# maybeLx/MVSFormerPlusPlus

Hardware: NVIDIA H100
Metric: depth-maps/sec (hot path: FMT + 4-stage cascade) (higher is better)
Workload: dtype f32

## Files before the change

include/mvsf_b200.h:

```cpp
#ifndef MVSF_B200_H
#define MVSF_B200_H

#include <stddef.h>
#include <stdint.h>

#ifdef __cplusplus
extern "C" {
#endif

typedef void* mvsf_stream_t;

enum mvsf_status {
  MVSF_OK = 0,
  MVSF_ERR_INVALID = -1,
  MVSF_ERR_CUDA = -2,
  MVSF_ERR_WORKSPACE = -3
};

const char* mvsf_last_error(void);
int mvsf_abi_version(void);
long long mvsf_launch_count(int reset);
int mvsf_ktimer_enable(int on);
int mvsf_ktimer_read(const char* name, double* ms, long long* launches);

int mvsf_nchw_to_nhwc(const float* src, float* dst, int N, int C, int HW, mvsf_stream_t stream);
int mvsf_nhwc_to_nchw(const float* src, float* dst, int N, int C, int HW, mvsf_stream_t stream);

int mvsf_compose_geometry(const float* proj, int V, float* homs, float* kinv_ref, mvsf_stream_t stream);

int mvsf_homography_from_proj(const float* src_proj, const float* ref_proj, int B, float* homs, mvsf_stream_t stream);

int mvsf_init_inverse_range(const float* depth_values, int Dn, float* out, int D, int H, int W, mvsf_stream_t stream);
int mvsf_schedule_inverse_range(const float* prev_depth, const float* prev_hypo, int Dp, float split_itv, float* out,
                                int D, int H, int W, mvsf_stream_t stream);
int mvsf_position3d(const float* kinv_ref, const float* depth, const float* depth_values, int Dn, float* stats,
                    int compute_minmax, float* pos, int D, int H, int W, mvsf_stream_t stream);

int mvsf_homo_warp(const float* src_nhwc, const float* hom, const float* depth, float* warped, uint8_t* mask, int C,
                   int D, int H, int W, mvsf_stream_t stream);

int mvsf_warp_corr_set_tile_path(int mode);
int mvsf_warp_corr_last_selection(int* used_pipeline, int* miss_permille);

int mvsf_warp_corr_plan(int C, int G, int D, int H, int W, int V, size_t spill_budget_bytes);

int mvsf_warp_corr_entropy(const float* feat, const float* homs, const float* depth, float* entropy, int V, int C,
                           int G, int D, int H, int W, mvsf_stream_t stream);
int mvsf_vis_cnn(const float* entropy, const float* wts, float* vis, int N, int H, int W, mvsf_stream_t stream);
int mvsf_warp_corr_aggregate(const float* feat, const float* homs, const float* depth, const float* vis,
                             float* volume, int V, int C, int G, int D, int H, int W, mvsf_stream_t stream);
int mvsf_warp_corr_entropy_store(const float* feat, const float* homs, const float* depth, float* entropy, float* corr,
                                 int V, int C, int G, int D, int H, int W, mvsf_stream_t stream);
int mvsf_corr_aggregate(const float* corr, const float* vis, float* volume, int V, int G, int D, int H, int W,
                        mvsf_stream_t stream);

int mvsf_costreg_unet_workspace_bytes(int kind, int C, int D, int H, int W, size_t* bytes);
int mvsf_costreg_unet_tc_bytes(size_t* bytes);
int mvsf_costreg_unet_pack_tc(int kind, const float* conv, void* wts_tc, size_t wts_tc_bytes, mvsf_stream_t stream);
int mvsf_costreg_unet_forward(int kind, const float* volume, const float* wts, const void* wts_tc, float* logits,
                              void* workspace, size_t workspace_bytes, int C, int D, int H, int W, mvsf_stream_t stream);
int mvsf_conv3d_tc_layer(int mode, int sd, const float* in, const float* w32, const float* skip, float* out,
                         void* workspace, size_t workspace_bytes, int cin, int cout, int ID, int IH, int IW,
                         mvsf_stream_t stream);

int mvsf_costreg_tr_workspace_bytes(int C, int D, int H, int W, size_t* bytes);
int mvsf_costreg_tr_forward(float* volume, const float* pos, const float* wts, const void* wts16, size_t n_wts,
                            float* logits, void* workspace, size_t workspace_bytes, int C, int D, int H, int W,
                            int layers, float softmax_scale, mvsf_stream_t stream);
int mvsf_split_weights_f16(const float* wts, void* out16, size_t n, mvsf_stream_t stream);

int mvsf_attention_forward(const float* qkv, float* out, void* workspace, size_t workspace_bytes, int N,
                           float softmax_scale, mvsf_stream_t stream);

int mvsf_attention_split_plan(int N, int num_sms, int* split_items, int* parts);

int mvsf_linear_tc_epilogue(int epi, const float* A, int lda, const float* W, const float* bias, const float* res,
                            int ldres, const float* gamma, const float* ln_w, const float* ln_b, float ln_eps,
                            int elu_cols, float* C, int ldc, float* Cpre, int ldcpre, void* C2, int ldc2,
                            void* workspace, size_t workspace_bytes, int M, int N, int K, mvsf_stream_t stream);
int mvsf_token_mlp_forward(int form, const float* A, const float* res, const float* proj_w, const float* proj_b,
                           const float* gamma1, const float* mid_w, const float* mid_b, float mid_eps, const float* f1_w,
                           const float* f1_b, const float* f2_w, const float* f2_b, const float* gamma2,
                           const float* out_w, const float* out_b, float out_eps, float* C, void* C2, void* workspace,
                           size_t workspace_bytes, int M, mvsf_stream_t stream);
int mvsf_linear_tc_streamed_epilogue(int epi, const float* A, int lda, const float* W, const float* bias,
                                     const float* res, int ldres, const float* gamma, int elu_cols, float* C, int ldc,
                                     void* C2, int ldc2, void* workspace, size_t workspace_bytes, int M, int N, int K,
                                     mvsf_stream_t stream);

int mvsf_softargmax(const float* logits, const float* depth_hypo, float tmp, float* prob, float* depth, float* conf,
                    int D, int H, int W, mvsf_stream_t stream);
int mvsf_conf_accumulate(const float* conf, int h, int w, float* acc, int H, int W, float scale, int init,
                         mvsf_stream_t stream);

int mvsf_fmt_workspace_bytes(int V, int H1, int W1, size_t* bytes);
int mvsf_fmt_forward(const float* f1, const float* f2, const float* f3, const float* f4, const float* pe,
                     const float* wts, const void* wts16, size_t n_wts, float* o1, float* o2, float* o3, float* o4,
                     void* workspace, size_t workspace_bytes, int V, int H1, int W1, mvsf_stream_t stream);

int mvsf_fpn_encoder_workspace_bytes(int N, int H, int W, size_t* bytes);
int mvsf_fpn_encoder_forward(const float* x, const float* wts, const void* wts_tc, float* c01, float* c11, float* c21,
                             float* c31, void* workspace, size_t workspace_bytes, int N, int H, int W, mvsf_stream_t stream);
int mvsf_fpn_encoder_vit_forward(const float* x, const float* vit_feat, int V, const float* wts, const void* wts_tc,
                                 float* c01, float* c11, float* c21, float* c31, void* workspace, size_t workspace_bytes,
                                 int N, int H, int W, mvsf_stream_t stream);
int mvsf_fpn_decoder_workspace_bytes(int N, int H, int W, size_t* bytes);
int mvsf_fpn_decoder_forward(const float* c01, const float* c11, const float* c21, const float* c31, const float* wts,
                             const void* wts_tc, float* o0, float* o1, float* o2, float* o3, void* workspace,
                             size_t workspace_bytes, int N, int H, int W, mvsf_stream_t stream);
int mvsf_fpn_tc_bytes(int part, size_t* bytes);
int mvsf_fpn_pack_tc(int part, const float* conv, void* wts_tc, size_t wts_tc_bytes, mvsf_stream_t stream);

int mvsf_vit_decoder_workspace_bytes(int B, int V, int h, int w, size_t* bytes);
int mvsf_vit_decoder_forward(const float* x0, const float* x1, const float* x2, const float* wts, const void* wts_tc,
                             float* out, void* workspace, size_t workspace_bytes, int B, int V, int h, int w,
                             mvsf_stream_t stream);

int mvsf_vit_workspace_bytes(int n, int gh, int gw, size_t* bytes);
int mvsf_vit_forward(const float* img, const float* pos, const float* wts, const void* wts_tc, float* out0, float* out1,
                     float* out2, void* workspace, size_t workspace_bytes, int n, int gh, int gw, mvsf_stream_t stream);
int mvsf_vit_forward_image(const float* img, int H, int W, const float* pos, const float* wts, const void* wts_tc,
                           float* out0, float* out1, float* out2, void* workspace, size_t workspace_bytes, int n, int gh,
                           int gw, mvsf_stream_t stream);
int mvsf_vit_attention_forward(const float* qkv, int ldq, float* out, int ldo, void* workspace, size_t workspace_bytes,
                               int n, int N, mvsf_stream_t stream);

int mvsf_fusion_workspace_bytes(int H, int W, size_t* bytes);
int mvsf_fusion_prepare_cameras(const float* cams, int N, float* cams_inv, mvsf_stream_t stream);
int mvsf_fusion_filter(int method, const float* depths, const float* confs, const float* cams, const float* cams_inv, int N,
                       int ref, const int* src, int V, int H, int W, float conf, float thres_view, float thres_disp,
                       float dist_base, float rel_diff_base, unsigned char* mask, float* depth_avg, void* workspace,
                       size_t workspace_bytes, mvsf_stream_t stream);
int mvsf_fusion_extract(const unsigned char* mask, const float* depth_avg, const void* workspace, size_t workspace_bytes,
                        const float* cam_inv, const float* image, float* xyz, unsigned char* rgb, long long capacity, int H,
                        int W, mvsf_stream_t stream);

#ifdef __cplusplus
}
#endif
#endif
```

mvsformerplusplus_b200/csrc/conv3d_tc.cu:

```cuda
#include "conv3d_tc.cuh"

#include <type_traits>

#include "linear_tc.cuh"
#include "wgmma.cuh"

namespace mvsf {

using namespace gmma;

namespace c3 {
constexpr int THREADS = 384, MAX_STAGES = 8;
template <int MODE, int NT>
struct Geo {
  static constexpr int TW = 8 * NT, TH = 16;
  static constexpr int PR = MODE == CONV_S1 ? TH + 2 : TH + 1;
  static constexpr int PC = MODE == CONV_S1 ? TW + 2 : TW + 1;
  static constexpr int NSUB = MODE == CONV_S2 ? 4 : 1;
  static constexpr uint32_t SUB_BYTES = PR * PC * 16;
  static constexpr uint32_t PAIR = (2 * SUB_BYTES + 127) / 128 * 128;
  static constexpr uint32_t OCT_BYTES = NSUB * PAIR;
  static constexpr uint32_t PITCH = PC * 16;
};
__host__ __device__ inline int npad(int cout) { return cout < 16 ? 16 : cout; }
__host__ __device__ inline uint32_t slab_bytes(int mode, int cout) { return (uint32_t)npad(cout) * (mode == DECONV_S2 ? 1024u : 576u); }

struct alignas(64) Maps { CUtensorMap m[4]; };
}

struct DepthTaps { int n, kd[3], id[3]; };
template <int MODE>
__device__ __forceinline__ DepthTaps depth_taps(int od, int SD, int ID) {
  DepthTaps t;
  t.n = 0;
#pragma unroll
  for (int kd = 0; kd < 3; ++kd) {
    int id;
    bool ok = true;
    if (MODE == CONV_S1) id = od + kd - 1;
    else if (MODE == CONV_S2) id = od * SD + kd - 1;
    else {
      const int num = od + 1 - kd;
      if (SD == 1) id = num;
      else { ok = (num & 1) == 0; id = num >> 1; }
    }
    if (ok && id >= 0 && id < ID) { t.kd[t.n] = kd; t.id[t.n] = id; ++t.n; }
  }
  return t;
}

template <int OUT, int NPAD>
__device__ __forceinline__ float conv_epilogue_frag(const ConvTcArgs& a, const float* acc, int h, int q, bool valid, size_t vox) {
  const int COUT = a.COUT;
  float prob = 0.f;
#pragma unroll
  for (int b = 0; b < NPAD / 8; ++b) {
    const int c = 8 * b + 2 * q;
    if (8 * b >= COUT) continue;
    const float2 b2 = *reinterpret_cast<const float2*>(a.bias + c);
    float x0 = fmaxf(acc[4 * b + 2 * h] + b2.x, 0.f), x1 = fmaxf(acc[4 * b + 2 * h + 1] + b2.y, 0.f);
    if (!valid) continue;
    if (OUT == OUT_SPLIT) {
      if (a.skip_hi) {
        const float2 fh = __half22float2(*reinterpret_cast<const __half2*>(a.skip_hi + vox * COUT + c));
        const float2 fl = __half22float2(*reinterpret_cast<const __half2*>(a.skip_lo + vox * COUT + c));
        x0 += fh.x + fl.x;
        x1 += fh.y + fl.y;
      }
      split_store2(a.out_hi + vox * COUT + c, a.out_lo + vox * COUT + c, x0, x1);
    } else {
      const float2 s2 = *reinterpret_cast<const float2*>(a.skip32 + vox * COUT + c);
      x0 += s2.x; x1 += s2.y;
      if (OUT == OUT_F32) *reinterpret_cast<float2*>(a.out32 + vox * COUT + c) = make_float2(x0, x1);
      else prob = fmaf(x1, __ldg(a.probw + c + 1), x0 * __ldg(a.probw + c));
    }
  }
  return prob;
}

template <int NREG>
__device__ __forceinline__ void fence_acc(float (&acc)[NREG]) { fence_regs<NREG>(acc); }

template <int MODE, int NT, int OUT, int NPAD>
__global__ void __launch_bounds__(c3::THREADS, 1)
conv3d_tc_kernel(const __grid_constant__ c3::Maps maps, ConvTcArgs a, int NS, int OD, int OH, int OW, int tiles_w,
                 int tiles_h, int ntiles) {
  using G = c3::Geo<MODE, NT>;
  constexpr int PC = G::PC, NSUB = G::NSUB;
  constexpr int NCLS = MODE == DECONV_S2 ? 4 : 1;
  constexpr int ACC = NCLS * NPAD / 2;
  extern __shared__ __align__(1024) unsigned char smem[];
  const int tid = threadIdx.x, warp = tid >> 5, lane = tid & 31;
  const int CIN = a.CIN, SD = a.SD, ID = a.ID, IH = a.IH, IW = a.IW;
  const int KG = a.KG;
  const uint32_t b_bytes = c3::slab_bytes(MODE, NPAD);
  const uint32_t a_bytes = (uint32_t)KG * G::OCT_BYTES;
  const uint32_t stage_bytes = (a_bytes + b_bytes + 127u) / 128u * 128u;
  const uint32_t sbase = smem_u32(smem);
  const uint32_t bars = sbase + NS * stage_bytes;
  const uint32_t bar_full = bars, bar_empty = bars + 64;
  const int ngroups = (CIN >> 3) / KG;

  if (tid == 0) {
    for (int i = 0; i < c3::MAX_STAGES; ++i) { mbar_init(bar_full + 8 * i, 1); mbar_init(bar_empty + 8 * i, 2); }
    fence_barrier_init();
  }
  __syncthreads();

  if (warp < 4) {
    asm volatile("setmaxnreg.dec.sync.aligned.u32 40;");
    if (tid == 0) {
      uint32_t g = 0;
      for (int tile = blockIdx.x; tile < ntiles; tile += gridDim.x) {
        const int tw = tile % tiles_w, th = (tile / tiles_w) % tiles_h, od = tile / (tiles_w * tiles_h);
        const int c0h = th * 16, c0w = tw * G::TW;
        const DepthTaps dt = depth_taps<MODE>(od, SD, ID);
        for (int ds = 0; ds < dt.n; ++ds) {
          for (int grp = 0; grp < ngroups; ++grp, ++g) {
            const int s = g % NS;
            mbar_wait(bar_empty + 8 * s, (uint32_t)(((g / NS) & 1) ^ 1));
            const uint32_t st = sbase + s * stage_bytes, full = bar_full + 8 * s;
            expect_tx(full, (uint32_t)(KG * NSUB) * 2u * G::SUB_BYTES + b_bytes);
            for (int og = 0; og < KG; ++og) {
              const int c = (grp * KG + og) * 8;
#pragma unroll
              for (int sub = 0; sub < NSUB; ++sub) {
                int w0, h0;
                if (MODE == CONV_S1) { w0 = c0w - 1; h0 = c0h - 1; }
                else if (MODE == CONV_S2) { w0 = c0w - (sub & 1); h0 = c0h - (sub >> 1); }
                else { w0 = c0w; h0 = c0h; }
                tma_load_5d(st + (uint32_t)(og * NSUB + sub) * G::PAIR, &maps.m[sub], c, w0, h0, dt.id[ds], 0, full);
              }
            }
            bulk_load(st + a_bytes, a.wtc + (size_t)(dt.kd[ds] * ngroups + grp) * (b_bytes / 2), b_bytes, full);
          }
        }
      }
    }
    return;
  }
  asm volatile("setmaxnreg.inc.sync.aligned.u32 232;");
  const int half = (warp >> 2) - 1, wq = warp & 3, q = lane & 3, t128 = tid & 127;
  const uint32_t blk = (uint32_t)NPAD * 32u;
  float acc[NT][ACC];
  auto release = [&](uint32_t gb) { if (t128 == 0) mbar_arrive(bar_empty + 8 * (gb % NS)); };
  uint32_t g = 0;
  for (int tile = blockIdx.x; tile < ntiles; tile += gridDim.x) {
    const int tw = tile % tiles_w, th = (tile / tiles_w) % tiles_h, od = tile / (tiles_w * tiles_h);
    const DepthTaps dt = depth_taps<MODE>(od, SD, ID);
    const int U = dt.n * ngroups;
    int pend = -1;
    for (int u = 0; u < U; ++u, ++g) {
      const int s = g % NS;
      mbar_wait(bar_full + 8 * s, (uint32_t)((g / NS) & 1));
      const uint32_t sA = sbase + s * stage_bytes + (uint32_t)half * 8u * G::PITCH, sB = sbase + s * stage_bytes + a_bytes;
      auto issue = [&](uint32_t aoff, int bstart, bool overwrite) {
        constexpr uint32_t n = (uint32_t)(NCLS * NPAD);
        const uint32_t t0 = sB + (uint32_t)bstart * 2u * blk, t1 = t0 + (uint32_t)NCLS * blk;
        const uint64_t b0 = make_desc(t0, n * 16u, 128), b1 = make_desc(t1, n * 16u, 128);
        if (KG == 1) {
#pragma unroll
          for (int t = 0; t < NT; ++t)
            mma_ss<n>(acc[t], make_desc(sA + aoff + t * 128, G::SUB_BYTES, G::PITCH), b0, overwrite ? 0u : 1u);
#pragma unroll
          for (int t = 0; t < NT; ++t)
            mma_ss<n>(acc[t], make_desc(sA + aoff + t * 128, G::SUB_BYTES, G::PITCH), b1, 1u);
        } else {
#pragma unroll
          for (int t = 0; t < NT; ++t)
            mma_ss<n>(acc[t], make_desc(sA + G::SUB_BYTES + aoff + t * 128, G::OCT_BYTES, G::PITCH), b0, overwrite ? 0u : 1u);
#pragma unroll
          for (int t = 0; t < NT; ++t)
            mma_ss<n>(acc[t], make_desc(sA + aoff + t * 128, G::OCT_BYTES, G::PITCH), b1, 1u);
#pragma unroll
          for (int t = 0; t < NT; ++t)
            mma_ss<n>(acc[t], make_desc(sA + aoff + t * 128, G::OCT_BYTES, G::PITCH), b0, 1u);
        }
      };
      wg_fence();
      if constexpr (MODE == DECONV_S2) {
        issue(0u, 0, u == 0);
        issue(16u, 4, false);
        issue((uint32_t)PC * 16u, 8, false);
        issue((uint32_t)(PC + 1) * 16u, 12, false);
      } else {
#pragma unroll
        for (int kh = 0; kh < 3; ++kh) {
#pragma unroll
          for (int kw = 0; kw < 3; ++kw) {
            int sub = 0, rs = kh, cs = kw;
            if (MODE == CONV_S2) {
              sub = (kh == 1 ? 0 : 2) + (kw == 1 ? 0 : 1);
              rs = kh == 2 ? 1 : 0; cs = kw == 2 ? 1 : 0;
            }
            issue((uint32_t)sub * G::PAIR + (uint32_t)(rs * PC + cs) * 16u, kh * 3 + kw, u == 0 && kh == 0 && kw == 0);
          }
        }
      }
      wg_commit();
      if (pend >= 0) {
        wg_wait<1>();
        release((uint32_t)pend);
      }
      pend = (int)g;
    }
    wg_wait<0>();
#pragma unroll
    for (int t = 0; t < NT; ++t) fence_acc(acc[t]);
    release((uint32_t)pend);
#pragma unroll
    for (int t = 0; t < NT; ++t)
#pragma unroll
      for (int cls = 0; cls < NCLS; ++cls)
#pragma unroll
        for (int h = 0; h < 2; ++h) {
          const int ch = th * 16 + 8 * half + 2 * wq + h;
          const int cw = tw * G::TW + t * 8 + (lane >> 2);
          int oh, ow;
          bool valid;
          if (MODE == DECONV_S2) { oh = 2 * ch + (cls >> 1); ow = 2 * cw + (cls & 1); valid = ch < IH && cw < IW; }
          else { oh = ch; ow = cw; valid = ch < OH && cw < OW; }
          const size_t vox = valid ? ((size_t)od * OH + oh) * OW + ow : 0;
          float prob = conv_epilogue_frag<OUT, NPAD>(a, acc[t] + (cls ^ (cls >> 1)) * (NPAD / 2), h, q, valid, vox);
          if (OUT == OUT_PROB) {
            prob += __shfl_xor_sync(0xffffffffu, prob, 1);
            prob += __shfl_xor_sync(0xffffffffu, prob, 2);
            if (q == 0 && valid) a.out32[vox] = prob + __ldg(a.probw + a.COUT);
          }
        }
  }
}


template <int MODE, int NT, int NPAD>
__global__ void __launch_bounds__(c3::THREADS, 1)
conv3d_col_kernel(const __grid_constant__ c3::Maps maps, ConvTcArgs a, int NS, int wres, int OH, int OW, int tiles_w,
                  int tiles_h, int DC, int nitems) {
  using G = c3::Geo<MODE, NT>;
  constexpr int PC = G::PC, NSUB = G::NSUB;
  extern __shared__ __align__(1024) unsigned char smem[];
  const int tid = threadIdx.x, warp = tid >> 5, lane = tid & 31;
  const int CIN = a.CIN, D = a.ID;
  const int KG = a.KG;
  const int ngroups = (CIN >> 3) / KG;
  const uint32_t slab = (uint32_t)NPAD * 1728u;
  const uint32_t a_bytes = (uint32_t)KG * G::OCT_BYTES;
  const uint32_t stage_bytes = (a_bytes + (wres ? 0u : slab) + 127u) / 128u * 128u;
  const uint32_t sbase = smem_u32(smem);
  const uint32_t wbase = sbase;
  const uint32_t ring = sbase + (wres ? ((uint32_t)ngroups * slab + 127u) / 128u * 128u : 0u);
  const uint32_t bars = ring + NS * stage_bytes;
  const uint32_t bar_full = bars, bar_empty = bars + 64, bar_w = bars + 128;

  if (tid == 0) {
    for (int i = 0; i < c3::MAX_STAGES; ++i) { mbar_init(bar_full + 8 * i, 1); mbar_init(bar_empty + 8 * i, 2); }
    mbar_init(bar_w, 1);
    fence_barrier_init();
  }
  __syncthreads();
  const int tiles_hw = tiles_w * tiles_h;

  if (warp < 4) {
    asm volatile("setmaxnreg.dec.sync.aligned.u32 40;");
    if (tid == 0) {
      if (wres) {
        expect_tx(bar_w, (uint32_t)ngroups * slab);
        for (int grp = 0; grp < ngroups; ++grp) bulk_load(wbase + grp * slab, a.wtc + (size_t)grp * (slab / 2), slab, bar_w);
      }
      uint32_t g = 0;
      for (int item = blockIdx.x; item < nitems; item += gridDim.x) {
        const int tw = item % tiles_w, th = (item / tiles_w) % tiles_h, ck = item / tiles_hw;
        const int c0h = th * 16, c0w = tw * G::TW;
        const int d0 = ck * DC, d1 = min(D, d0 + DC);
        const int first_id = max(d0 - 1, 0), last_id = min(d1, D - 1);
        for (int id = first_id; id <= last_id; ++id) {
          for (int grp = 0; grp < ngroups; ++grp, ++g) {
            const int s = g % NS;
            mbar_wait(bar_empty + 8 * s, (uint32_t)(((g / NS) & 1) ^ 1));
            const uint32_t st = ring + s * stage_bytes, full = bar_full + 8 * s;
            expect_tx(full, (uint32_t)(KG * NSUB) * 2u * G::SUB_BYTES + (wres ? 0u : slab));
            for (int og = 0; og < KG; ++og) {
              const int c = (grp * KG + og) * 8;
#pragma unroll
              for (int sub = 0; sub < NSUB; ++sub) {
                int w0, h0;
                if (MODE == CONV_S1) { w0 = c0w - 1; h0 = c0h - 1; }
                else { w0 = c0w - (sub & 1); h0 = c0h - (sub >> 1); }
                tma_load_5d(st + (uint32_t)(og * NSUB + sub) * G::PAIR, &maps.m[sub], c, w0, h0, id, 0, full);
              }
            }
            if (!wres) bulk_load(st + a_bytes, a.wtc + (size_t)grp * (slab / 2), slab, full);
          }
        }
      }
    }
    return;
  }
  asm volatile("setmaxnreg.inc.sync.aligned.u32 232;");
  const int half = (warp >> 2) - 1, wq = warp & 3, q = lane & 3, t128 = tid & 127;
  if (wres) mbar_wait(bar_w, 0u);
  constexpr uint32_t btile = (uint32_t)NPAD * 96u;
  constexpr uint32_t blbo = (uint32_t)NPAD * 48u;
  constexpr int SL = NPAD / 2;
  float acc[NT][3 * SL];
  auto release = [&](uint32_t gb) { if (t128 == 0) mbar_arrive(bar_empty + 8 * (gb % NS)); };
  auto epilogue = [&](int od, int th, int tw, auto third_c) {
#pragma unroll
    for (int t = 0; t < NT; ++t)
#pragma unroll
      for (int h = 0; h < 2; ++h) {
        const int ch = th * 16 + 8 * half + 2 * wq + h;
        const int cw = tw * G::TW + t * 8 + (lane >> 2);
        const bool valid = ch < OH && cw < OW;
        const size_t vox = valid ? ((size_t)od * OH + ch) * OW + cw : 0;
        conv_epilogue_frag<OUT_SPLIT, NPAD>(a, acc[t] + decltype(third_c)::value * SL, h, q, valid, vox);
      }
  };
  uint32_t g = 0;
  for (int item = blockIdx.x; item < nitems; item += gridDim.x) {
    const int tw = item % tiles_w, th = (item / tiles_w) % tiles_h, ck = item / tiles_hw;
    const int d0 = ck * DC, d1 = min(D, d0 + DC);
    const int first_id = max(d0 - 1, 0), last_id = min(d1, D - 1);
#pragma unroll
    for (int t = 0; t < NT; ++t)
#pragma unroll
      for (int i = 0; i < 3 * SL; ++i) acc[t][i] = 0.f;
    for (int id = first_id; id <= last_id; ++id) {
      int pend = -1;
      for (int grp = 0; grp < ngroups; ++grp, ++g) {
        const int s = g % NS;
        mbar_wait(bar_full + 8 * s, (uint32_t)((g / NS) & 1));
        const uint32_t sA = ring + s * stage_bytes + (uint32_t)half * 8u * G::PITCH;
        const uint32_t sB = wres ? wbase + grp * slab : ring + s * stage_bytes + a_bytes;
        wg_fence();
#pragma unroll
        for (int kh = 0; kh < 3; ++kh) {
#pragma unroll
          for (int kw = 0; kw < 3; ++kw) {
            int sub = 0, rs = kh, cs = kw;
            if (MODE == CONV_S2) {
              sub = (kh == 1 ? 0 : 2) + (kw == 1 ? 0 : 1);
              rs = kh == 2 ? 1 : 0; cs = kw == 2 ? 1 : 0;
            }
            const uint32_t aoff = sA + (uint32_t)sub * G::PAIR + (uint32_t)(rs * PC + cs) * 16u;
            const uint32_t t0 = sB + (uint32_t)(kh * 3 + kw) * 2u * btile, t1 = t0 + btile;
            const uint32_t va[3] = {KG == 1 ? aoff : aoff + G::SUB_BYTES, KG == 1 ? aoff : aoff, aoff};
            const uint32_t vl = KG == 1 ? G::SUB_BYTES : G::OCT_BYTES;
            const uint32_t vt[3] = {t0, t1, t0};
            const int nv = KG == 1 ? 2 : 3;
#pragma unroll
            for (int v = 0; v < 3; ++v) {
              if (v >= nv) break;
              const uint64_t bd = make_desc(vt[v], blbo, 128);
#pragma unroll
              for (int t = 0; t < NT; ++t) mma_ss<3 * NPAD>(acc[t], make_desc(va[v] + t * 128, vl, G::PITCH), bd, 1u);
            }
          }
        }
        wg_commit();
        if (pend >= 0) {
          wg_wait<1>();
          release((uint32_t)pend);
        }
        pend = (int)g;
      }
      wg_wait<0>();
#pragma unroll
      for (int t = 0; t < NT; ++t) fence_acc(acc[t]);
      release((uint32_t)pend);
      if (id - 1 >= d0) epilogue(id - 1, th, tw, std::integral_constant<int, 0>{});
      if (id == last_id && id <= d1 - 1) epilogue(id, th, tw, std::integral_constant<int, 1>{});
#pragma unroll
      for (int t = 0; t < NT; ++t)
#pragma unroll
        for (int i = 0; i < SL; ++i) {
          acc[t][i] = acc[t][SL + i];
          acc[t][SL + i] = acc[t][2 * SL + i];
          acc[t][2 * SL + i] = 0.f;
        }
    }
  }
}

int conv3d_tc_kg(int mode, int cin) { return (mode != CONV_S2 && cin >= 16) ? 2 : 1; }
int conv3d_tc_col(int mode, int sd, int cout) { return (mode == CONV_S1 || (mode == CONV_S2 && sd == 1)) && c3::npad(cout) <= 32; }

size_t conv3d_tc_packed_halves(int mode, int cin, int cout) {
  return (size_t)3 * (cin / 8 / conv3d_tc_kg(mode, cin)) * (c3::slab_bytes(mode, cout) / 2);
}

__global__ void conv3d_tc_pack_kernel(const float* __restrict__ w32, __half* __restrict__ out, int cin, int cout, int NPAD,
                                      int KG, int deconv, int col, size_t total) {
  size_t i = (size_t)blockIdx.x * blockDim.x + threadIdx.x;
  if (i >= total) return;
  const int e = (int)(i & 7);
  const size_t q = i >> 3;
  const int per_slab = col ? NPAD * 108 : (deconv ? NPAD * 64 : NPAD * 36);
  const int slab = (int)(q / per_slab), c = (int)(q % per_slab);
  const int ngroups = cin / 8 / KG;
  int kd = slab / ngroups, g = slab % ngroups;
  int mm, kc, n, kh = 0, kw = 0;
  bool tap = true;
  if (col) {
    g = slab;
    n = c % NPAD;
    int r = c / NPAD;
    kd = 2 - r % 3; r /= 3;
    kc = r & 1; r >>= 1;
    mm = r & 1; r >>= 1;
    kh = r / 3; kw = r % 3;
  } else if (!deconv) {
    n = c % NPAD;
    int r = c / NPAD;
    kc = r & 1; r >>= 1;
    mm = r & 1; r >>= 1;
    kh = r / 3; kw = r % 3;
  } else {
    const int tkh[4][4] = {{1, 1, 2, 2}, {-1, 1, 2, -1}, {-1, -1, 0, 0}, {-1, -1, 0, -1}};
    const int tkw[4][4] = {{1, 2, 2, 1}, {-1, 0, 0, -1}, {-1, -1, 2, 1}, {-1, -1, 0, -1}};
    const int t = c / (16 * NPAD), cc = c % (16 * NPAD);
    mm = cc / (8 * NPAD);
    kc = (cc / (4 * NPAD)) & 1;
    const int nn = cc % (4 * NPAD);
    const int b = nn / NPAD;
    n = nn % NPAD;
    kh = tkh[t][b]; kw = tkw[t][b];
    tap = kh >= 0;
  }
  const int ci = (KG == 1 ? g : g * 2 + kc) * 8 + e;
  float w = 0.f;
  if (tap && n < cout) w = w32[((size_t)((kd * 3 + kh) * 3 + kw) * cin + ci) * cout + n];
  __half hi, lo;
  split_f16(w, hi, lo);
  __half v;
  if (KG == 1) v = mm == 0 ? hi : (kc == 0 ? lo : __float2half_rn(0.f));
  else v = mm == 0 ? hi : lo;
  out[i] = v;
}

int conv3d_tc_pack(const float* w32, __half* out, int mode, int sd, int cin, int cout, cudaStream_t s) {
  MVSF_REQUIRE(w32 && out && cin % 8 == 0 && cout % 8 == 0, "conv3d_tc_pack: bad arguments");
  const size_t total = conv3d_tc_packed_halves(mode, cin, cout);
  conv3d_tc_pack_kernel<<<cdiv((long long)total, 256), 256, 0, s>>>(w32, out, cin, cout, c3::npad(cout),
                                                                     conv3d_tc_kg(mode, cin), mode == DECONV_S2 ? 1 : 0,
                                                                     conv3d_tc_col(mode, sd, cout), total);
  MVSF_LAUNCH_CHECK("conv3d_tc_pack");
  return MVSF_OK;
}

__global__ void merge_vec8_kernel(const __half* __restrict__ hi, const __half* __restrict__ lo, float* __restrict__ x, size_t n8) {
  size_t i = (size_t)blockIdx.x * blockDim.x + threadIdx.x;
  if (i >= n8) return;
  const uint4 h = *reinterpret_cast<const uint4*>(hi + i * 8), l = *reinterpret_cast<const uint4*>(lo + i * 8);
  const __half2* h2 = reinterpret_cast<const __half2*>(&h);
  const __half2* l2 = reinterpret_cast<const __half2*>(&l);
  float r[8];
#pragma unroll
  for (int e = 0; e < 4; ++e) {
    const float2 fh = __half22float2(h2[e]), fl = __half22float2(l2[e]);
    r[2 * e] = fh.x + fl.x;
    r[2 * e + 1] = fh.y + fl.y;
  }
  *reinterpret_cast<float4*>(x + i * 8) = make_float4(r[0], r[1], r[2], r[3]);
  *reinterpret_cast<float4*>(x + i * 8 + 4) = make_float4(r[4], r[5], r[6], r[7]);
}
int launch_merge_vec8(const __half* hi, const __half* lo, float* x, size_t n, cudaStream_t s) {
  MVSF_REQUIRE(x && hi && lo && n > 0 && n % 8 == 0, "merge_vec8: bad arguments");
  merge_vec8_kernel<<<cdiv((long long)(n / 8), 256), 256, 0, s>>>(hi, lo, x, n / 8);
  MVSF_LAUNCH_CHECK("merge_vec8");
  return MVSF_OK;
}

static int make_map(CUtensorMap* m, const __half* hi, const __half* lo, int C, int D, int H, int W, int sh, int sw, int ph,
                    int pw, int box_w, int box_h) {
  EncodeTiledFn enc = encode_tiled_fn();
  MVSF_REQUIRE(enc, "conv3d_tc: cuTensorMapEncodeTiled is not available from this driver");
  const long long lo_off = (lo - hi) * (long long)sizeof(__half);
  MVSF_REQUIRE(lo_off > 0 && lo_off % 16 == 0, "conv3d_tc: the lo tensor must follow the hi tensor at a 16-byte multiple");
  const cuuint64_t dims[5] = {(cuuint64_t)C, (cuuint64_t)((W - pw + sw - 1) / sw), (cuuint64_t)((H - ph + sh - 1) / sh), (cuuint64_t)D, 2};
  const cuuint64_t strides[4] = {(cuuint64_t)sw * C * 2, (cuuint64_t)sh * W * C * 2, (cuuint64_t)H * W * C * 2, (cuuint64_t)lo_off};
  const cuuint32_t box[5] = {8, (cuuint32_t)box_w, (cuuint32_t)box_h, 1, 2};
  const cuuint32_t estr[5] = {1, 1, 1, 1, 1};
  void* base = const_cast<__half*>(hi + ((size_t)ph * W + pw) * C);
  CUresult r = enc(m, CU_TENSOR_MAP_DATA_TYPE_FLOAT16, 5, base, dims, strides, box, estr, CU_TENSOR_MAP_INTERLEAVE_NONE,
                   CU_TENSOR_MAP_SWIZZLE_NONE, CU_TENSOR_MAP_L2_PROMOTION_L2_128B, CU_TENSOR_MAP_FLOAT_OOB_FILL_NONE);
  if (r != CUDA_SUCCESS) return fail(MVSF_ERR_CUDA, "conv3d_tc: cuTensorMapEncodeTiled failed (%d) for C=%d D=%d H=%d W=%d", (int)r, C, D, H, W);
  return MVSF_OK;
}

template <int MODE, int NT, int OUT, int NPAD>
static int launch_one(const ConvTcArgs& a, int NS, size_t smem, int OD, int OH, int OW, int cells_h, int cells_w,
                      int num_sms, cudaStream_t s) {
  using G = c3::Geo<MODE, NT>;
  auto kern = conv3d_tc_kernel<MODE, NT, OUT, NPAD>;
  static DeviceOnce once;
  const int dev = current_device();
  if (once.need(dev)) {
    MVSF_CUDA_OK(cudaFuncSetAttribute(kern, cudaFuncAttributeMaxDynamicSharedMemorySize, 227 * 1024));
    once.done(dev);
  }
  c3::Maps maps;
  int rc;
  if (MODE == CONV_S2) {
    for (int sub = 0; sub < 4; ++sub)
      if ((rc = make_map(&maps.m[sub], a.in_hi, a.in_lo, a.CIN, a.ID, a.IH, a.IW, 2, 2, sub >> 1, sub & 1, G::PC, G::PR))) return rc;
  } else {
    if ((rc = make_map(&maps.m[0], a.in_hi, a.in_lo, a.CIN, a.ID, a.IH, a.IW, 1, 1, 0, 0, G::PC, G::PR))) return rc;
    maps.m[1] = maps.m[2] = maps.m[3] = maps.m[0];
  }
  const int tiles_w = cdiv(cells_w, 8 * NT), tiles_h = cdiv(cells_h, 16);
  const long long ntiles = (long long)tiles_w * tiles_h * OD;
  MVSF_REQUIRE(ntiles < (1ll << 30), "conv3d_tc: volume too large");
  const int grid = (int)(ntiles < num_sms ? ntiles : num_sms);
  kern<<<grid, c3::THREADS, smem, s>>>(maps, a, NS, OD, OH, OW, tiles_w, tiles_h, (int)ntiles);
  MVSF_LAUNCH_CHECK("conv3d_tc");
  return MVSF_OK;
}

template <int MODE, int OUT, int NPAD>
static int launch_nt(const ConvTcArgs& a, int nt, int NS, size_t smem, int OD, int OH, int OW, int cells_h, int cells_w,
                     int num_sms, cudaStream_t s) {
  constexpr int NCLS = MODE == DECONV_S2 ? 4 : 1;
  if constexpr (4 * NCLS * NPAD <= 256)
    if (nt == 4) return launch_one<MODE, 4, OUT, NPAD>(a, NS, smem, OD, OH, OW, cells_h, cells_w, num_sms, s);
  if constexpr (2 * NCLS * NPAD <= 256)
    if (nt == 2) return launch_one<MODE, 2, OUT, NPAD>(a, NS, smem, OD, OH, OW, cells_h, cells_w, num_sms, s);
  return launch_one<MODE, 1, OUT, NPAD>(a, NS, smem, OD, OH, OW, cells_h, cells_w, num_sms, s);
}

template <int MODE, int OUT>
static int launch_mode(const ConvTcArgs& a, cudaStream_t s) {
  int OD, OH, OW, cells_h, cells_w;
  if (MODE == CONV_S1) { OD = a.ID; OH = a.IH; OW = a.IW; cells_h = OH; cells_w = OW; }
  else if (MODE == CONV_S2) { OD = (a.ID - 1) / a.SD + 1; OH = (a.IH - 1) / 2 + 1; OW = (a.IW - 1) / 2 + 1; cells_h = OH; cells_w = OW; }
  else { OD = a.ID * a.SD; OH = a.IH * 2; OW = a.IW * 2; cells_h = a.IH; cells_w = a.IW; }
  const int num_sms = device_sm_count(current_device());
  const int NPAD = c3::npad(a.COUT);
  const uint32_t b_bytes = c3::slab_bytes(MODE, a.COUT);
  const int ncls = MODE == DECONV_S2 ? 4 : 1;
  int best_nt = 0;
  double best_eff = -1.0;
  const int nts[3] = {4, 2, 1};
  size_t stage_of[5] = {0, 0, 0, 0, 0};
  for (int k = 0; k < 3; ++k) {
    const int nt = nts[k];
    const uint32_t oct = nt == 4 ? c3::Geo<MODE, 4>::OCT_BYTES : (nt == 2 ? c3::Geo<MODE, 2>::OCT_BYTES : c3::Geo<MODE, 1>::OCT_BYTES);
    const size_t stage = align_up((size_t)a.KG * oct + b_bytes, 128);
    stage_of[nt] = stage;
    if (nt * ncls * NPAD > 256 || 2 * stage + 256 > 227 * 1024) continue;
    const long long ntiles = (long long)cdiv(cells_w, 8 * nt) * cdiv(cells_h, 16) * OD;
    const double eff = (double)ntiles / (double)(cdiv(ntiles, num_sms) * (long long)num_sms);
    if (eff >= 0.85) { best_nt = nt; break; }
    if (eff > best_eff) { best_eff = eff; best_nt = nt; }
  }
  MVSF_REQUIRE(best_nt > 0, "conv3d_tc: no tile shape fits (COUT %d)", a.COUT);
  const size_t stage = stage_of[best_nt];
  int NS = (int)((227 * 1024 - 256) / stage);
  if (NS > c3::MAX_STAGES) NS = c3::MAX_STAGES;
  const size_t smem = NS * stage + 256;
  if constexpr (OUT == OUT_SPLIT) {
    if (NPAD == 32) return launch_nt<MODE, OUT, 32>(a, best_nt, NS, smem, OD, OH, OW, cells_h, cells_w, num_sms, s);
    if (NPAD == 64) return launch_nt<MODE, OUT, 64>(a, best_nt, NS, smem, OD, OH, OW, cells_h, cells_w, num_sms, s);
  }
  return launch_nt<MODE, OUT, 16>(a, best_nt, NS, smem, OD, OH, OW, cells_h, cells_w, num_sms, s);
}


template <int MODE, int NT, int NPAD>
static int launch_col_one(const ConvTcArgs& a, int NS, int wres, size_t smem, int OH, int OW, int DC, int num_sms, cudaStream_t s) {
  using G = c3::Geo<MODE, NT>;
  auto kern = conv3d_col_kernel<MODE, NT, NPAD>;
  static DeviceOnce once;
  const int dev = current_device();
  if (once.need(dev)) {
    MVSF_CUDA_OK(cudaFuncSetAttribute(kern, cudaFuncAttributeMaxDynamicSharedMemorySize, 227 * 1024));
    once.done(dev);
  }
  c3::Maps maps;
  int rc;
  if (MODE == CONV_S2) {
    for (int sub = 0; sub < 4; ++sub)
      if ((rc = make_map(&maps.m[sub], a.in_hi, a.in_lo, a.CIN, a.ID, a.IH, a.IW, 2, 2, sub >> 1, sub & 1, G::PC, G::PR))) return rc;
  } else {
    if ((rc = make_map(&maps.m[0], a.in_hi, a.in_lo, a.CIN, a.ID, a.IH, a.IW, 1, 1, 0, 0, G::PC, G::PR))) return rc;
    maps.m[1] = maps.m[2] = maps.m[3] = maps.m[0];
  }
  const int tiles_w = cdiv(OW, 8 * NT), tiles_h = cdiv(OH, 16);
  const long long nitems = (long long)tiles_w * tiles_h * cdiv(a.ID, DC);
  MVSF_REQUIRE(nitems < (1ll << 30), "conv3d_tc: volume too large");
  const int grid = (int)(nitems < num_sms ? nitems : num_sms);
  kern<<<grid, c3::THREADS, smem, s>>>(maps, a, NS, wres, OH, OW, tiles_w, tiles_h, DC, (int)nitems);
  MVSF_LAUNCH_CHECK("conv3d_col");
  return MVSF_OK;
}

template <int MODE>
static int launch_col(const ConvTcArgs& a, cudaStream_t s) {
  const int D = a.ID;
  const int OH = MODE == CONV_S1 ? a.IH : (a.IH - 1) / 2 + 1, OW = MODE == CONV_S1 ? a.IW : (a.IW - 1) / 2 + 1;
  const int num_sms = device_sm_count(current_device());
  const int NPAD = c3::npad(a.COUT);
  const int ngroups = a.CIN / 8 / a.KG;
  const size_t slab = (size_t)NPAD * 1728;
  const size_t wres_bytes = align_up(ngroups * slab, 128);
  const int wres = wres_bytes <= 112 * 1024 ? 1 : 0;
  int best_nt = 0, best_dc = 0, best_ns = 0;
  size_t best_smem = 0;
  double best_cost = 1e30;
  const int nts[3] = {4, 2, 1};
  for (int k = 0; k < 3; ++k) {
    const int nt = nts[k];
    if (3 * nt * NPAD > 128) continue;
    const uint32_t oct = nt == 4 ? c3::Geo<MODE, 4>::OCT_BYTES : (nt == 2 ? c3::Geo<MODE, 2>::OCT_BYTES : c3::Geo<MODE, 1>::OCT_BYTES);
    const size_t stage = align_up((size_t)a.KG * oct + (wres ? 0 : slab), 128);
    const size_t fixed = (wres ? wres_bytes : 0) + 256;
    int ns = (int)((227 * 1024 - fixed) / stage);
    if (ns > c3::MAX_STAGES) ns = c3::MAX_STAGES;
    if (ns < 2) continue;
    for (int div = 1; div <= 8; div *= 2) {
      const int dc = cdiv(D, div);
      if (div > 1 && dc == cdiv(D, div / 2)) continue;
      const long long items = (long long)cdiv(OW, 8 * nt) * cdiv(OH, 16) * cdiv(D, dc);
      const double eff = (double)items / (double)(cdiv(items, num_sms) * (long long)num_sms);
      const double halo_w = MODE == CONV_S1 ? (8.0 * nt + 2) / (8.0 * nt) : (16.0 * nt + 1) / (16.0 * nt);
      const double halo_d = dc >= D ? 1.0 : (dc + 2.0) / dc;
      const double cost = halo_w * halo_d / eff;
      if (cost < best_cost) { best_cost = cost; best_nt = nt; best_dc = dc; best_ns = ns; best_smem = fixed + ns * stage; }
    }
  }
  MVSF_REQUIRE(best_nt > 0, "conv3d_col: no tile shape fits (CIN %d COUT %d)", a.CIN, a.COUT);
  if (NPAD == 16) {
    if (best_nt == 2) return launch_col_one<MODE, 2, 16>(a, best_ns, wres, best_smem, OH, OW, best_dc, num_sms, s);
    return launch_col_one<MODE, 1, 16>(a, best_ns, wres, best_smem, OH, OW, best_dc, num_sms, s);
  }
  return launch_col_one<MODE, 1, 32>(a, best_ns, wres, best_smem, OH, OW, best_dc, num_sms, s);
}

int launch_conv3d_tc(const ConvTcArgs& a, int mode, int out_mode, cudaStream_t s) {
  MVSF_REQUIRE(a.in_hi && a.in_lo && a.wtc && a.bias, "conv3d_tc: null pointer");
  MVSF_REQUIRE(a.CIN % 8 == 0 && a.CIN >= 8 && a.CIN <= 64 && (a.COUT == 8 || a.COUT == 16 || a.COUT == 32 || a.COUT == 64),
               "conv3d_tc: input channels must be a multiple of 8 up to 64, output channels 8, 16, 32 or 64");
  MVSF_REQUIRE(a.SD == 1 || a.SD == 2, "conv3d_tc: depth stride must be 1 or 2");
  MVSF_REQUIRE(a.KG == conv3d_tc_kg(mode, a.CIN), "conv3d_tc: KG must be conv3d_tc_kg(mode, CIN) (it fixes the weight slab layout)");
  MVSF_REQUIRE(((uintptr_t)a.in_hi & 15) == 0 && ((uintptr_t)a.in_lo & 15) == 0 && ((uintptr_t)a.wtc & 15) == 0,
               "conv3d_tc: operands must be 16-byte aligned");
  MVSF_REQUIRE(a.col == conv3d_tc_col(mode, a.SD, a.COUT), "conv3d_tc: col must be conv3d_tc_col(mode, SD, COUT) (weight slab layout)");
  if (out_mode == OUT_SPLIT) {
    MVSF_REQUIRE(a.out_hi && a.out_lo, "conv3d_tc: split output missing");
    if (a.col) return mode == CONV_S1 ? launch_col<CONV_S1>(a, s) : launch_col<CONV_S2>(a, s);
    if (mode == CONV_S1) return launch_mode<CONV_S1, OUT_SPLIT>(a, s);
    if (mode == CONV_S2) return launch_mode<CONV_S2, OUT_SPLIT>(a, s);
    if (mode == DECONV_S2) return launch_mode<DECONV_S2, OUT_SPLIT>(a, s);
  } else if (mode == DECONV_S2 && (out_mode == OUT_F32 || out_mode == OUT_PROB)) {
    MVSF_REQUIRE(a.out32 && a.skip32 && a.COUT == 8 && (out_mode == OUT_F32 || a.probw), "conv3d_tc: fp32 output needs out32, skip32, COUT == 8");
    if (out_mode == OUT_F32) return launch_mode<DECONV_S2, OUT_F32>(a, s);
    return launch_mode<DECONV_S2, OUT_PROB>(a, s);
  }
  return fail(MVSF_ERR_INVALID, "conv3d_tc: unsupported mode %d / output %d", mode, out_mode);
}

}

using namespace mvsf;

extern "C" int mvsf_conv3d_tc_layer(int mode, int sd, const float* in, const float* w32, const float* skip, float* out,
                                    void* workspace, size_t workspace_bytes, int cin, int cout, int ID, int IH, int IW,
                                    mvsf_stream_t stream) {
  MVSF_REQUIRE(in && w32 && out && workspace && (mode >= 0 && mode <= 2) && (sd == 1 || sd == 2), "conv3d_tc_layer: bad arguments");
  MVSF_REQUIRE(cin % 8 == 0 && cout % 8 == 0, "conv3d_tc_layer: channels must be multiples of 8");
  int OD, OH, OW;
  if (mode == CONV_S1) { OD = ID; OH = IH; OW = IW; }
  else if (mode == CONV_S2) { OD = (ID - 1) / sd + 1; OH = (IH - 1) / 2 + 1; OW = (IW - 1) / 2 + 1; }
  else { OD = ID * sd; OH = IH * 2; OW = IW * 2; }
  const size_t nin = (size_t)ID * IH * IW * cin, nout = (size_t)OD * OH * OW * cout;
  const size_t nw = align_up(conv3d_tc_packed_halves(mode, cin, cout), 64);
  const size_t need = (2 * nin + 4 * nout + nw) * sizeof(__half) + 256;
  if (workspace_bytes < need) return fail(MVSF_ERR_WORKSPACE, "conv3d_tc_layer: workspace %zu < %zu bytes", workspace_bytes, need);
  cudaStream_t s = (cudaStream_t)stream;
  __half* xin = reinterpret_cast<__half*>(workspace);
  __half* xout = xin + 2 * nin;
  __half* xskip = xout + 2 * nout;
  __half* wtc = xskip + 2 * nout;
  int rc;
  if ((rc = launch_split_f16(in, nin, xin, 2 * nin, 1, nin, s))) return rc;
  if (skip && (rc = launch_split_f16(skip, nout, xskip, 2 * nout, 1, nout, s))) return rc;
  if ((rc = conv3d_tc_pack(w32, wtc, mode, sd, cin, cout, s))) return rc;
  ConvTcArgs a{};
  a.in_hi = xin; a.in_lo = xin + nin; a.wtc = wtc; a.bias = w32 + (size_t)27 * cin * cout;
  if (skip) { a.skip_hi = xskip; a.skip_lo = xskip + nout; }
  a.out_hi = xout; a.out_lo = xout + nout;
  a.CIN = cin; a.COUT = cout; a.SD = sd; a.ID = ID; a.IH = IH; a.IW = IW; a.KG = conv3d_tc_kg(mode, cin);
  a.col = conv3d_tc_col(mode, sd, cout);
  if ((rc = launch_conv3d_tc(a, mode, OUT_SPLIT, s))) return rc;
  return launch_merge_vec8(xout, xout + nout, out, nout, s);
}
```

mvsformerplusplus_b200/csrc/conv3d_tc.cuh:

```cuda
#pragma once
#include <cuda_fp16.h>

#include "common.cuh"

namespace mvsf {

enum ConvTcMode { CONV_S1 = 0, CONV_S2 = 1, DECONV_S2 = 2 };
enum ConvTcOut { OUT_SPLIT = 0, OUT_F32 = 1, OUT_PROB = 2 };

struct ConvTcArgs {
  const __half* in_hi; const __half* in_lo;
  const __half* wtc;
  const float* bias;
  const __half* skip_hi; const __half* skip_lo;
  const float* skip32;
  __half* out_hi; __half* out_lo;
  float* out32;
  const float* probw;
  int CIN, COUT, SD, ID, IH, IW;
  int KG;
  int col;
};

int conv3d_tc_kg(int mode, int cin);
size_t conv3d_tc_packed_halves(int mode, int cin, int cout);
int conv3d_tc_col(int mode, int sd, int cout);
int conv3d_tc_pack(const float* w32, __half* out, int mode, int sd, int cin, int cout, cudaStream_t s);
int launch_conv3d_tc(const ConvTcArgs& a, int mode, int out_mode, cudaStream_t s);
int launch_merge_vec8(const __half* hi, const __half* lo, float* x, size_t n, cudaStream_t s);

}
```

mvsformerplusplus_b200/csrc/costreg_unet.cu:

```cuda
#include "common.cuh"
#include "conv3d_tc.cuh"

namespace mvsf {

__global__ void prob3_kernel(const float* __restrict__ in, const float* __restrict__ w, float* __restrict__ out, int D,
                             int H, int W) {
  __shared__ float ws[27 * 8];
  for (int i = threadIdx.x; i < 27 * 8; i += blockDim.x) ws[i] = __ldg(w + i);
  __syncthreads();
  int x = blockIdx.x * blockDim.x + threadIdx.x, y = blockIdx.y, d = blockIdx.z;
  if (x >= W) return;
  float acc = 0.f;
  for (int kd = 0; kd < 3; ++kd) {
    int zd = d + kd - 1;
    if (zd < 0 || zd >= D) continue;
    for (int kh = 0; kh < 3; ++kh) {
      int yh = y + kh - 1;
      if (yh < 0 || yh >= H) continue;
#pragma unroll
      for (int kw = 0; kw < 3; ++kw) {
        int xw = x + kw - 1;
        if (xw < 0 || xw >= W) continue;
        const float* p = in + (((size_t)zd * H + yh) * W + xw) * 8;
        float4 a = ldg4(p), b = ldg4(p + 4);
        const float* wp = ws + ((kd * 3 + kh) * 3 + kw) * 8;
        acc = fmaf(a.x, wp[0], acc); acc = fmaf(a.y, wp[1], acc); acc = fmaf(a.z, wp[2], acc); acc = fmaf(a.w, wp[3], acc);
        acc = fmaf(b.x, wp[4], acc); acc = fmaf(b.y, wp[5], acc); acc = fmaf(b.z, wp[6], acc); acc = fmaf(b.w, wp[7], acc);
      }
    }
  }
  out[((size_t)d * H + y) * W + x] = acc;
}

constexpr int kLayerCh[9][2] = {{8, 16}, {16, 16}, {16, 32}, {32, 32}, {32, 64}, {64, 64}, {64, 32}, {32, 16}, {16, 8}};
static const int kLayerMode[9] = {CONV_S2, CONV_S1, CONV_S2, CONV_S1, CONV_S2, CONV_S1, DECONV_S2, DECONV_S2, DECONV_S2};

constexpr size_t unet_floats(bool conv) {
  size_t n = 0;
  for (int l = 0; l < 9; ++l) n += conv ? (size_t)27 * kLayerCh[l][0] * kLayerCh[l][1] : kLayerCh[l][1];
  return n;
}
constexpr size_t NCONV = unet_floats(true), NSMALL[2] = {unet_floats(false) + 27 * 8, unet_floats(false) + 8 + 1 + 3};
static_assert(NCONV == 290304 && NSMALL[0] == 496 && NSMALL[1] == 292,
              "packing.COSTREG_UNET_CONV_WTS / COSTREG_UNET_SMALL_WTS");

static size_t tc_total_halves() {
  size_t n = 0;
  for (int l = 0; l < 9; ++l) n += conv3d_tc_packed_halves(kLayerMode[l], kLayerCh[l][0], kLayerCh[l][1]);
  return n;
}

static int unet_forward_tc(int kind, const float* vol, const float* wts, const __half* wtc, float* logits, void* ws, int D,
                           int H, int W, cudaStream_t s) {
  const int SD = kind == 0 ? 2 : 1;
  const int D1 = (D - 1) / SD + 1, H1 = H / 2, W1 = W / 2;
  const int D2 = (D1 - 1) / SD + 1, H2 = H1 / 2, W2 = W1 / 2;
  const int D3 = (D2 - 1) / SD + 1, H3 = H2 / 2, W3 = W2 / 2;
  const size_t n0 = (size_t)D * H * W * 8;
  const size_t n1 = (size_t)D1 * H1 * W1 * 16, n2 = (size_t)D2 * H2 * W2 * 32, n3 = (size_t)D3 * H3 * W3 * 64;
  __half* v0 = reinterpret_cast<__half*>(ws);
  __half* t1 = v0 + 2 * n0;   __half* c2 = t1 + 2 * n1;
  __half* t3 = c2 + 2 * n1;   __half* c4 = t3 + 2 * n2;
  __half* t5 = c4 + 2 * n2;   __half* c6 = t5 + 2 * n3;
  float* x11 = reinterpret_cast<float*>(c6 + 2 * n3);
  const float* bias[9];
  const __half* w16[9];
  {
    const float* p = wts;
    const __half* q = wtc;
    for (int l = 0; l < 9; ++l) {
      bias[l] = p; w16[l] = q;
      p += kLayerCh[l][1];
      q += conv3d_tc_packed_halves(kLayerMode[l], kLayerCh[l][0], kLayerCh[l][1]);
    }
  }
  const float* wp = bias[8] + 8;
  int rc;
  if ((rc = launch_split_f16(vol, n0, v0, 2 * n0, 1, n0, s))) return rc;
  auto conv = [&](int l, const __half* in, size_t nin, __half* out, size_t nout, const __half* skip, size_t nskip,
                  int ID, int IH, int IW) {
    ConvTcArgs a{};
    a.in_hi = in; a.in_lo = in + nin;
    a.wtc = w16[l]; a.bias = bias[l];
    a.skip_hi = skip; a.skip_lo = skip ? skip + nskip : nullptr;
    a.out_hi = out; a.out_lo = out + nout;
    a.CIN = kLayerCh[l][0]; a.COUT = kLayerCh[l][1]; a.SD = SD; a.ID = ID; a.IH = IH; a.IW = IW;
    a.KG = conv3d_tc_kg(kLayerMode[l], a.CIN);
    a.col = conv3d_tc_col(kLayerMode[l], SD, a.COUT);
    return launch_conv3d_tc(a, kLayerMode[l], OUT_SPLIT, s);
  };
  if ((rc = conv(0, v0, n0, t1, n1, nullptr, 0, D, H, W))) return rc;
  if ((rc = conv(1, t1, n1, c2, n1, nullptr, 0, D1, H1, W1))) return rc;
  if ((rc = conv(2, c2, n1, t3, n2, nullptr, 0, D1, H1, W1))) return rc;
  if ((rc = conv(3, t3, n2, c4, n2, nullptr, 0, D2, H2, W2))) return rc;
  if ((rc = conv(4, c4, n2, t5, n3, nullptr, 0, D2, H2, W2))) return rc;
  if ((rc = conv(5, t5, n3, c6, n3, nullptr, 0, D3, H3, W3))) return rc;
  if ((rc = conv(6, c6, n3, t3, n2, c4, n2, D3, H3, W3))) return rc;
  if ((rc = conv(7, t3, n2, t1, n1, c2, n1, D2, H2, W2))) return rc;
  {
    ConvTcArgs a{};
    a.in_hi = t1; a.in_lo = t1 + n1;
    a.wtc = w16[8]; a.bias = bias[8];
    a.skip32 = vol;
    a.CIN = 16; a.COUT = 8; a.SD = SD; a.ID = D1; a.IH = H1; a.IW = W1; a.KG = conv3d_tc_kg(DECONV_S2, 16);
    if (kind == 1) {
      a.out32 = logits; a.probw = wp;
      if ((rc = launch_conv3d_tc(a, DECONV_S2, OUT_PROB, s))) return rc;
    } else {
      a.out32 = x11;
      if ((rc = launch_conv3d_tc(a, DECONV_S2, OUT_F32, s))) return rc;
      dim3 grid(cdiv(W, 128), H, D);
      prob3_kernel<<<grid, 128, 0, s>>>(x11, wp, logits, D, H, W);
      MVSF_LAUNCH_CHECK("prob3");
    }
  }
  return MVSF_OK;
}

}

using namespace mvsf;

extern "C" {

int mvsf_costreg_unet_workspace_bytes(int kind, int C, int D, int H, int W, size_t* bytes) {
  MVSF_REQUIRE(bytes && (kind == 0 || kind == 1) && C == 8, "costreg_unet: kind in {0,1}, C == 8");
  MVSF_REQUIRE(H % 8 == 0 && W % 8 == 0 && D >= 1 && (kind == 1 || D % 8 == 0),
               "costreg_unet: H, W (and D for CostRegNet) must be multiples of 8");
  const int SD = kind == 0 ? 2 : 1;
  size_t D1 = (D - 1) / SD + 1, D2 = (D1 - 1) / SD + 1, D3 = (D2 - 1) / SD + 1;
  size_t n1 = D1 * (H / 2) * (W / 2) * 16, n2 = D2 * (H / 4) * (W / 4) * 32, n3 = D3 * (H / 8) * (W / 8) * 64;
  size_t n = (size_t)D * H * W * 8 + 2 * (n1 + n2 + n3) + (kind == 0 ? (size_t)D * H * W * 8 : 0);
  *bytes = n * sizeof(float);
  return MVSF_OK;
}

int mvsf_costreg_unet_tc_bytes(size_t* bytes) {
  MVSF_REQUIRE(bytes, "costreg_unet_tc_bytes: null pointer");
  *bytes = tc_total_halves() * sizeof(__half);
  return MVSF_OK;
}

int mvsf_costreg_unet_pack_tc(int kind, const float* conv, void* wts_tc, size_t wts_tc_bytes, mvsf_stream_t stream) {
  MVSF_REQUIRE(conv && wts_tc && ((uintptr_t)wts_tc & 15) == 0 && (kind == 0 || kind == 1), "costreg_unet_pack_tc: null or unaligned pointer, or bad kind");
  if (wts_tc_bytes < tc_total_halves() * sizeof(__half))
    return fail(MVSF_ERR_WORKSPACE, "costreg_unet_pack_tc: buffer %zu < %zu bytes", wts_tc_bytes, tc_total_halves() * sizeof(__half));
  const float* p = conv;
  __half* q = reinterpret_cast<__half*>(wts_tc);
  for (int l = 0; l < 9; ++l) {
    int rc = conv3d_tc_pack(p, q, kLayerMode[l], kind == 0 ? 2 : 1, kLayerCh[l][0], kLayerCh[l][1], (cudaStream_t)stream);
    if (rc) return rc;
    p += (size_t)27 * kLayerCh[l][0] * kLayerCh[l][1];
    q += conv3d_tc_packed_halves(kLayerMode[l], kLayerCh[l][0], kLayerCh[l][1]);
  }
  return MVSF_OK;
}

int mvsf_costreg_unet_forward(int kind, const float* volume, const float* wts, const void* wts_tc, float* logits,
                              void* workspace, size_t workspace_bytes, int C, int D, int H, int W, mvsf_stream_t stream) {
  MVSF_REQUIRE(volume && wts && logits && workspace, "costreg_unet: null pointer");
  size_t need = 0;
  int rc = mvsf_costreg_unet_workspace_bytes(kind, C, D, H, W, &need);
  if (rc) return rc;
  if (workspace_bytes < need) return fail(MVSF_ERR_WORKSPACE, "costreg_unet: workspace %zu < %zu bytes", workspace_bytes, need);
  MVSF_REQUIRE(((uintptr_t)workspace & 15) == 0 && ((uintptr_t)wts & 15) == 0 && ((uintptr_t)volume & 15) == 0,
               "costreg_unet: pointers must be 16-byte aligned");
  MVSF_REQUIRE(wts_tc && ((uintptr_t)wts_tc & 15) == 0, "costreg_unet: wts_tc (mvsf_costreg_unet_pack_tc) is required, 16-byte aligned");
  return unet_forward_tc(kind, volume, wts, reinterpret_cast<const __half*>(wts_tc), logits, workspace, D, H, W,
                         (cudaStream_t)stream);
}
}
```

Measured before the change: 51.09.

## Extend depth-streaming column conv kernel to transposed stride-2 final layer

Adds a DECONV_S2 path to the depth-streaming column kernel. The final 16->8 transposed conv in the unet, with fp32 skip and fused prob/F32 output, now streams input depth slices in reverse and accumulates all four output parity classes with one pass of the A tile per slice, instead of re-reading inputs per output slice. The epilogue is deferred and its skip loads are issued after the next group's MMAs are committed, so they overlap tensor-core work. Weight packing gains a matching column layout for deconv. The cost is more accumulator registers and complexity.

```diff
diff --git a/include/mvsf_b200.h b/include/mvsf_b200.h
--- a/include/mvsf_b200.h
+++ b/include/mvsf_b200.h
@@ -62,6 +62,9 @@
 int mvsf_conv3d_tc_layer(int mode, int sd, const float* in, const float* w32, const float* skip, float* out,
                          void* workspace, size_t workspace_bytes, int cin, int cout, int ID, int IH, int IW,
                          mvsf_stream_t stream);
+int mvsf_conv3d_tc_layer_out(int mode, int sd, int out_mode, int col, const float* in, const float* w32,
+                             const float* skip, const float* probw, float* out, void* workspace, size_t workspace_bytes,
+                             int cin, int cout, int ID, int IH, int IW, mvsf_stream_t stream);
 
 int mvsf_costreg_tr_workspace_bytes(int C, int D, int H, int W, size_t* bytes);
 int mvsf_costreg_tr_forward(float* volume, const float* pos, const float* wts, const void* wts16, size_t n_wts,
diff --git a/mvsformerplusplus_b200/csrc/conv3d_tc.cu b/mvsformerplusplus_b200/csrc/conv3d_tc.cu
--- a/mvsformerplusplus_b200/csrc/conv3d_tc.cu
+++ b/mvsformerplusplus_b200/csrc/conv3d_tc.cu
@@ -49,8 +49,37 @@
   return t;
 }
 
+template <int MODE>
+__device__ __forceinline__ size_t cell_vox(const ConvTcArgs& a, int od, int ch, int cw, int cls, int OH, int OW, bool& valid) {
+  int oh = ch, ow = cw;
+  if (MODE == DECONV_S2) { oh = 2 * ch + (cls >> 1); ow = 2 * cw + (cls & 1); valid = ch < a.IH && cw < a.IW; }
+  else valid = ch < OH && cw < OW;
+  return valid ? ((size_t)od * OH + oh) * OW + ow : 0;
+}
+
 template <int OUT, int NPAD>
-__device__ __forceinline__ float conv_epilogue_frag(const ConvTcArgs& a, const float* acc, int h, int q, bool valid, size_t vox) {
+__device__ __forceinline__ void load_skip(const ConvTcArgs& a, int q, bool valid, size_t vox, float2 (&sk)[NPAD / 8]) {
+  const int COUT = a.COUT;
+#pragma unroll
+  for (int b = 0; b < NPAD / 8; ++b) {
+    const int c = 8 * b + 2 * q;
+    sk[b] = make_float2(0.f, 0.f);
+    if (8 * b >= COUT || !valid) continue;
+    if (OUT == OUT_SPLIT) {
+      if (a.skip_hi) {
+        const float2 fh = __half22float2(*reinterpret_cast<const __half2*>(a.skip_hi + vox * COUT + c));
+        const float2 fl = __half22float2(*reinterpret_cast<const __half2*>(a.skip_lo + vox * COUT + c));
+        sk[b] = make_float2(fh.x + fl.x, fh.y + fl.y);
+      }
+    } else {
+      sk[b] = *reinterpret_cast<const float2*>(a.skip32 + vox * COUT + c);
+    }
+  }
+}
+
+template <int OUT, int NPAD>
+__device__ __forceinline__ float conv_epilogue_frag(const ConvTcArgs& a, const float* acc, const float2 (&sk)[NPAD / 8], int h,
+                                                    int q, bool valid, size_t vox) {
   const int COUT = a.COUT;
   float prob = 0.f;
 #pragma unroll
@@ -62,20 +91,28 @@
     if (!valid) continue;
     if (OUT == OUT_SPLIT) {
       if (a.skip_hi) {
-        const float2 fh = __half22float2(*reinterpret_cast<const __half2*>(a.skip_hi + vox * COUT + c));
-        const float2 fl = __half22float2(*reinterpret_cast<const __half2*>(a.skip_lo + vox * COUT + c));
-        x0 += fh.x + fl.x;
-        x1 += fh.y + fl.y;
+        x0 += sk[b].x;
+        x1 += sk[b].y;
       }
       split_store2(a.out_hi + vox * COUT + c, a.out_lo + vox * COUT + c, x0, x1);
     } else {
-      const float2 s2 = *reinterpret_cast<const float2*>(a.skip32 + vox * COUT + c);
-      x0 += s2.x; x1 += s2.y;
+      x0 += sk[b].x; x1 += sk[b].y;
       if (OUT == OUT_F32) *reinterpret_cast<float2*>(a.out32 + vox * COUT + c) = make_float2(x0, x1);
       else prob = fmaf(x1, __ldg(a.probw + c + 1), x0 * __ldg(a.probw + c));
     }
   }
   return prob;
+}
+
+template <int OUT, int NPAD>
+__device__ __forceinline__ void cell_epilogue(const ConvTcArgs& a, const float* acc, const float2 (&sk)[NPAD / 8], size_t vox,
+                                              bool valid, int cls, int h, int q) {
+  float prob = conv_epilogue_frag<OUT, NPAD>(a, acc + (cls ^ (cls >> 1)) * (NPAD / 2), sk, h, q, valid, vox);
+  if (OUT == OUT_PROB) {
+    prob += __shfl_xor_sync(0xffffffffu, prob, 1);
+    prob += __shfl_xor_sync(0xffffffffu, prob, 2);
+    if (q == 0 && valid) a.out32[vox] = prob + __ldg(a.probw + a.COUT);
+  }
 }
 
 template <int NREG>
@@ -91,7 +128,7 @@
   constexpr int ACC = NCLS * NPAD / 2;
   extern __shared__ __align__(1024) unsigned char smem[];
   const int tid = threadIdx.x, warp = tid >> 5, lane = tid & 31;
-  const int CIN = a.CIN, SD = a.SD, ID = a.ID, IH = a.IH, IW = a.IW;
+  const int CIN = a.CIN, SD = a.SD, ID = a.ID;
   const int KG = a.KG;
   const uint32_t b_bytes = c3::slab_bytes(MODE, NPAD);
   const uint32_t a_bytes = (uint32_t)KG * G::OCT_BYTES;
@@ -214,36 +251,33 @@
       for (int cls = 0; cls < NCLS; ++cls)
 #pragma unroll
         for (int h = 0; h < 2; ++h) {
-          const int ch = th * 16 + 8 * half + 2 * wq + h;
-          const int cw = tw * G::TW + t * 8 + (lane >> 2);
-          int oh, ow;
           bool valid;
-          if (MODE == DECONV_S2) { oh = 2 * ch + (cls >> 1); ow = 2 * cw + (cls & 1); valid = ch < IH && cw < IW; }
-          else { oh = ch; ow = cw; valid = ch < OH && cw < OW; }
-          const size_t vox = valid ? ((size_t)od * OH + oh) * OW + ow : 0;
-          float prob = conv_epilogue_frag<OUT, NPAD>(a, acc[t] + (cls ^ (cls >> 1)) * (NPAD / 2), h, q, valid, vox);
-          if (OUT == OUT_PROB) {
-            prob += __shfl_xor_sync(0xffffffffu, prob, 1);
-            prob += __shfl_xor_sync(0xffffffffu, prob, 2);
-            if (q == 0 && valid) a.out32[vox] = prob + __ldg(a.probw + a.COUT);
-          }
-        }
-  }
-}
-
-
-template <int MODE, int NT, int NPAD>
+          const size_t vox = cell_vox<MODE>(a, od, th * 16 + 8 * half + 2 * wq + h, tw * G::TW + t * 8 + (lane >> 2), cls,
+                                            OH, OW, valid);
+          float2 sk[NPAD / 8];
+          load_skip<OUT, NPAD>(a, q, valid, vox, sk);
+          cell_epilogue<OUT, NPAD>(a, acc[t], sk, vox, valid, cls, h, q);
+        }
+  }
+}
+
+
+template <int MODE, int NT, int OUT, int NPAD>
 __global__ void __launch_bounds__(c3::THREADS, 1)
-conv3d_col_kernel(const __grid_constant__ c3::Maps maps, ConvTcArgs a, int NS, int wres, int OH, int OW, int tiles_w,
-                  int tiles_h, int DC, int nitems) {
+conv3d_col_kernel(const __grid_constant__ c3::Maps maps, ConvTcArgs a, int NS, int wres, int cells_h, int cells_w,
+                  int tiles_w, int tiles_h, int DC, int nitems) {
   using G = c3::Geo<MODE, NT>;
   constexpr int PC = G::PC, NSUB = G::NSUB;
+  constexpr bool DEC = MODE == DECONV_S2;
+  constexpr int NCLS = DEC ? 4 : 1;
+  constexpr int NBLK = DEC ? 4 : 9;
   extern __shared__ __align__(1024) unsigned char smem[];
   const int tid = threadIdx.x, warp = tid >> 5, lane = tid & 31;
   const int CIN = a.CIN, D = a.ID;
   const int KG = a.KG;
   const int ngroups = (CIN >> 3) / KG;
-  const uint32_t slab = (uint32_t)NPAD * 1728u;
+  const int OH = DEC ? 2 * cells_h : cells_h, OW = DEC ? 2 * cells_w : cells_w;
+  const uint32_t slab = (uint32_t)(NBLK * NCLS * NPAD) * 192u;
   const uint32_t a_bytes = (uint32_t)KG * G::OCT_BYTES;
   const uint32_t stage_bytes = (a_bytes + (wres ? 0u : slab) + 127u) / 128u * 128u;
   const uint32_t sbase = smem_u32(smem);
@@ -273,7 +307,8 @@
         const int c0h = th * 16, c0w = tw * G::TW;
         const int d0 = ck * DC, d1 = min(D, d0 + DC);
         const int first_id = max(d0 - 1, 0), last_id = min(d1, D - 1);
-        for (int id = first_id; id <= last_id; ++id) {
+        for (int k = 0; k <= last_id - first_id; ++k) {
+          const int id = DEC ? last_id - k : first_id + k;
           for (int grp = 0; grp < ngroups; ++grp, ++g) {
             const int s = g % NS;
             mbar_wait(bar_empty + 8 * s, (uint32_t)(((g / NS) & 1) ^ 1));
@@ -285,7 +320,8 @@
               for (int sub = 0; sub < NSUB; ++sub) {
                 int w0, h0;
                 if (MODE == CONV_S1) { w0 = c0w - 1; h0 = c0h - 1; }
-                else { w0 = c0w - (sub & 1); h0 = c0h - (sub >> 1); }
+                else if (MODE == CONV_S2) { w0 = c0w - (sub & 1); h0 = c0h - (sub >> 1); }
+                else { w0 = c0w; h0 = c0h; }
                 tma_load_5d(st + (uint32_t)(og * NSUB + sub) * G::PAIR, &maps.m[sub], c, w0, h0, id, 0, full);
               }
             }
@@ -299,22 +335,50 @@
   asm volatile("setmaxnreg.inc.sync.aligned.u32 232;");
   const int half = (warp >> 2) - 1, wq = warp & 3, q = lane & 3, t128 = tid & 127;
   if (wres) mbar_wait(bar_w, 0u);
-  constexpr uint32_t btile = (uint32_t)NPAD * 96u;
-  constexpr uint32_t blbo = (uint32_t)NPAD * 48u;
-  constexpr int SL = NPAD / 2;
-  float acc[NT][3 * SL];
+  constexpr int NH = DEC ? 2 : 1;
+  constexpr uint32_t N = (uint32_t)(3 * NCLS / NH * NPAD);
+  constexpr uint32_t btile = N * 32u;
+  constexpr uint32_t blbo = N * 16u;
+  constexpr int SLH = NCLS / NH * NPAD / 2;
+  constexpr int SL = NH * SLH;
+  float acc[NT][NH][3 * SLH];
+  float ep[NT][SL];
+  int ep_od = -1;
   auto release = [&](uint32_t gb) { if (t128 == 0) mbar_arrive(bar_empty + 8 * (gb % NS)); };
-  auto epilogue = [&](int od, int th, int tw, auto third_c) {
+  auto complete = [&](int od, auto third_c) {
 #pragma unroll
     for (int t = 0; t < NT; ++t)
 #pragma unroll
-      for (int h = 0; h < 2; ++h) {
-        const int ch = th * 16 + 8 * half + 2 * wq + h;
-        const int cw = tw * G::TW + t * 8 + (lane >> 2);
-        const bool valid = ch < OH && cw < OW;
-        const size_t vox = valid ? ((size_t)od * OH + ch) * OW + cw : 0;
-        conv_epilogue_frag<OUT_SPLIT, NPAD>(a, acc[t] + decltype(third_c)::value * SL, h, q, valid, vox);
-      }
+      for (int x = 0; x < NH; ++x)
+#pragma unroll
+        for (int i = 0; i < SLH; ++i) ep[t][x * SLH + i] = acc[t][x][decltype(third_c)::value * SLH + i];
+    ep_od = od;
+  };
+  auto flush = [&](int th, int tw) {
+    float2 sk[NT][NCLS][2][NPAD / 8];
+#pragma unroll
+    for (int t = 0; t < NT; ++t)
+#pragma unroll
+      for (int cls = 0; cls < NCLS; ++cls)
+#pragma unroll
+        for (int h = 0; h < 2; ++h) {
+          bool valid;
+          const size_t vox = cell_vox<MODE>(a, ep_od, th * 16 + 8 * half + 2 * wq + h, tw * G::TW + t * 8 + (lane >> 2),
+                                            cls, OH, OW, valid);
+          load_skip<OUT, NPAD>(a, q, valid, vox, sk[t][cls][h]);
+        }
+#pragma unroll
+    for (int t = 0; t < NT; ++t)
+#pragma unroll
+      for (int cls = 0; cls < NCLS; ++cls)
+#pragma unroll
+        for (int h = 0; h < 2; ++h) {
+          bool valid;
+          const size_t vox = cell_vox<MODE>(a, ep_od, th * 16 + 8 * half + 2 * wq + h, tw * G::TW + t * 8 + (lane >> 2),
+                                            cls, OH, OW, valid);
+          cell_epilogue<OUT, NPAD>(a, ep[t], sk[t][cls][h], vox, valid, cls, h, q);
+        }
+    ep_od = -1;
   };
   uint32_t g = 0;
   for (int item = blockIdx.x; item < nitems; item += gridDim.x) {
@@ -324,8 +388,11 @@
 #pragma unroll
     for (int t = 0; t < NT; ++t)
 #pragma unroll
-      for (int i = 0; i < 3 * SL; ++i) acc[t][i] = 0.f;
-    for (int id = first_id; id <= last_id; ++id) {
+      for (int x = 0; x < NH; ++x)
+#pragma unroll
+        for (int i = 0; i < 3 * SLH; ++i) acc[t][x][i] = 0.f;
+    for (int k = 0; k <= last_id - first_id; ++k) {
+      const int id = DEC ? last_id - k : first_id + k;
       int pend = -1;
       for (int grp = 0; grp < ngroups; ++grp, ++g) {
         const int s = g % NS;
@@ -334,30 +401,33 @@
         const uint32_t sB = wres ? wbase + grp * slab : ring + s * stage_bytes + a_bytes;
         wg_fence();
 #pragma unroll
-        for (int kh = 0; kh < 3; ++kh) {
-#pragma unroll
-          for (int kw = 0; kw < 3; ++kw) {
-            int sub = 0, rs = kh, cs = kw;
-            if (MODE == CONV_S2) {
-              sub = (kh == 1 ? 0 : 2) + (kw == 1 ? 0 : 1);
-              rs = kh == 2 ? 1 : 0; cs = kw == 2 ? 1 : 0;
-            }
-            const uint32_t aoff = sA + (uint32_t)sub * G::PAIR + (uint32_t)(rs * PC + cs) * 16u;
-            const uint32_t t0 = sB + (uint32_t)(kh * 3 + kw) * 2u * btile, t1 = t0 + btile;
-            const uint32_t va[3] = {KG == 1 ? aoff : aoff + G::SUB_BYTES, KG == 1 ? aoff : aoff, aoff};
-            const uint32_t vl = KG == 1 ? G::SUB_BYTES : G::OCT_BYTES;
-            const uint32_t vt[3] = {t0, t1, t0};
-            const int nv = KG == 1 ? 2 : 3;
-#pragma unroll
-            for (int v = 0; v < 3; ++v) {
-              if (v >= nv) break;
-              const uint64_t bd = make_desc(vt[v], blbo, 128);
-#pragma unroll
-              for (int t = 0; t < NT; ++t) mma_ss<3 * NPAD>(acc[t], make_desc(va[v] + t * 128, vl, G::PITCH), bd, 1u);
+        for (int b = 0; b < NBLK; ++b) {
+          int sub = 0, rs = DEC ? b >> 1 : b / 3, cs = DEC ? b & 1 : b % 3;
+          if (MODE == CONV_S2) {
+            const int kh = b / 3, kw = b % 3;
+            sub = (kh == 1 ? 0 : 2) + (kw == 1 ? 0 : 1);
+            rs = kh == 2 ? 1 : 0; cs = kw == 2 ? 1 : 0;
+          }
+          const uint32_t aoff = sA + (uint32_t)sub * G::PAIR + (uint32_t)(rs * PC + cs) * 16u;
+          const uint32_t t0 = sB + (uint32_t)b * 2u * NH * btile, t1 = t0 + NH * btile;
+          const uint32_t va[3] = {KG == 1 ? aoff : aoff + G::SUB_BYTES, KG == 1 ? aoff : aoff, aoff};
+          const uint32_t vl = KG == 1 ? G::SUB_BYTES : G::OCT_BYTES;
+          const uint32_t vt[3] = {t0, t1, t0};
+          const int nv = KG == 1 ? 2 : 3;
+#pragma unroll
+          for (int v = 0; v < 3; ++v) {
+            if (v >= nv) break;
+#pragma unroll
+            for (int x = 0; x < NH; ++x) {
+              if (DEC && x == 0 && b >= 2) continue;
+              const uint64_t bd = make_desc(vt[v] + (uint32_t)x * btile, blbo, 128);
+#pragma unroll
+              for (int t = 0; t < NT; ++t) mma_ss<N>(acc[t][x], make_desc(va[v] + t * 128, vl, G::PITCH), bd, 1u);
             }
           }
         }
         wg_commit();
+        if (grp == 0 && ep_od >= 0) flush(th, tw);
         if (pend >= 0) {
           wg_wait<1>();
           release((uint32_t)pend);
@@ -366,24 +436,38 @@
       }
       wg_wait<0>();
 #pragma unroll
-      for (int t = 0; t < NT; ++t) fence_acc(acc[t]);
+      for (int t = 0; t < NT; ++t)
+#pragma unroll
+        for (int x = 0; x < NH; ++x) fence_acc(acc[t][x]);
       release((uint32_t)pend);
-      if (id - 1 >= d0) epilogue(id - 1, th, tw, std::integral_constant<int, 0>{});
-      if (id == last_id && id <= d1 - 1) epilogue(id, th, tw, std::integral_constant<int, 1>{});
+      const int od = DEC ? id + 1 : id - 1;
+      if (DEC ? od <= d1 - 1 : od >= d0) complete(od, std::integral_constant<int, 0>{});
+      if (k == last_id - first_id) {
+        if (ep_od >= 0) flush(th, tw);
+        if (DEC ? id >= d0 : id <= d1 - 1) {
+          complete(id, std::integral_constant<int, 1>{});
+          flush(th, tw);
+        }
+      }
 #pragma unroll
       for (int t = 0; t < NT; ++t)
 #pragma unroll
-        for (int i = 0; i < SL; ++i) {
-          acc[t][i] = acc[t][SL + i];
-          acc[t][SL + i] = acc[t][2 * SL + i];
-          acc[t][2 * SL + i] = 0.f;
-        }
+        for (int x = 0; x < NH; ++x)
+#pragma unroll
+          for (int i = 0; i < SLH; ++i) {
+            acc[t][x][i] = acc[t][x][SLH + i];
+            acc[t][x][SLH + i] = acc[t][x][2 * SLH + i];
+            acc[t][x][2 * SLH + i] = 0.f;
+          }
     }
   }
 }
 
 int conv3d_tc_kg(int mode, int cin) { return (mode != CONV_S2 && cin >= 16) ? 2 : 1; }
-int conv3d_tc_col(int mode, int sd, int cout) { return (mode == CONV_S1 || (mode == CONV_S2 && sd == 1)) && c3::npad(cout) <= 32; }
+int conv3d_tc_col(int mode, int sd, int cout) {
+  if (mode == DECONV_S2) return sd == 1 && c3::npad(cout) <= 16;
+  return (mode == CONV_S1 || (mode == CONV_S2 && sd == 1)) && c3::npad(cout) <= 32;
+}
 
 size_t conv3d_tc_packed_halves(int mode, int cin, int cout) {
   return (size_t)3 * (cin / 8 / conv3d_tc_kg(mode, cin)) * (c3::slab_bytes(mode, cout) / 2);
@@ -395,13 +479,26 @@
   if (i >= total) return;
   const int e = (int)(i & 7);
   const size_t q = i >> 3;
-  const int per_slab = col ? NPAD * 108 : (deconv ? NPAD * 64 : NPAD * 36);
+  const int per_slab = col ? (deconv ? NPAD * 192 : NPAD * 108) : (deconv ? NPAD * 64 : NPAD * 36);
   const int slab = (int)(q / per_slab), c = (int)(q % per_slab);
   const int ngroups = cin / 8 / KG;
   int kd = slab / ngroups, g = slab % ngroups;
   int mm, kc, n, kh = 0, kw = 0;
   bool tap = true;
-  if (col) {
+  const int tkh[4][4] = {{1, 1, 2, 2}, {-1, 1, 2, -1}, {-1, -1, 0, 0}, {-1, -1, 0, -1}};
+  const int tkw[4][4] = {{1, 2, 2, 1}, {-1, 0, 0, -1}, {-1, -1, 2, 1}, {-1, -1, 0, -1}};
+  if (col && deconv) {
+    g = slab;
+    n = c % NPAD;
+    int r = c / NPAD;
+    const int bb = r & 1; r >>= 1;
+    kd = 2 - r % 3; r /= 3;
+    kc = r & 1; r >>= 1;
+    const int b = 2 * (r & 1) + bb; r >>= 1;
+    mm = r & 1; r >>= 1;
+    kh = tkh[r][b]; kw = tkw[r][b];
+    tap = kh >= 0;
+  } else if (col) {
     g = slab;
     n = c % NPAD;
     int r = c / NPAD;
@@ -416,8 +513,6 @@
     mm = r & 1; r >>= 1;
     kh = r / 3; kw = r % 3;
   } else {
-    const int tkh[4][4] = {{1, 1, 2, 2}, {-1, 1, 2, -1}, {-1, -1, 0, 0}, {-1, -1, 0, -1}};
-    const int tkw[4][4] = {{1, 2, 2, 1}, {-1, 0, 0, -1}, {-1, -1, 2, 1}, {-1, -1, 0, -1}};
     const int t = c / (16 * NPAD), cc = c % (16 * NPAD);
     mm = cc / (8 * NPAD);
     kc = (cc / (4 * NPAD)) & 1;
@@ -438,12 +533,12 @@
   out[i] = v;
 }
 
-int conv3d_tc_pack(const float* w32, __half* out, int mode, int sd, int cin, int cout, cudaStream_t s) {
-  MVSF_REQUIRE(w32 && out && cin % 8 == 0 && cout % 8 == 0, "conv3d_tc_pack: bad arguments");
+int conv3d_tc_pack(const float* w32, __half* out, int mode, int col, int cin, int cout, cudaStream_t s) {
+  MVSF_REQUIRE(w32 && out && cin % 8 == 0 && cout % 8 == 0 && (col == 0 || col == 1), "conv3d_tc_pack: bad arguments");
   const size_t total = conv3d_tc_packed_halves(mode, cin, cout);
   conv3d_tc_pack_kernel<<<cdiv((long long)total, 256), 256, 0, s>>>(w32, out, cin, cout, c3::npad(cout),
                                                                      conv3d_tc_kg(mode, cin), mode == DECONV_S2 ? 1 : 0,
-                                                                     conv3d_tc_col(mode, sd, cout), total);
+                                                                     col, total);
   MVSF_LAUNCH_CHECK("conv3d_tc_pack");
   return MVSF_OK;
 }
@@ -566,10 +661,11 @@
 }
 
 
-template <int MODE, int NT, int NPAD>
-static int launch_col_one(const ConvTcArgs& a, int NS, int wres, size_t smem, int OH, int OW, int DC, int num_sms, cudaStream_t s) {
+template <int MODE, int NT, int OUT, int NPAD>
+static int launch_col_one(const ConvTcArgs& a, int NS, int wres, size_t smem, int cells_h, int cells_w, int DC, int num_sms,
+                          cudaStream_t s) {
   using G = c3::Geo<MODE, NT>;
-  auto kern = conv3d_col_kernel<MODE, NT, NPAD>;
+  auto kern = conv3d_col_kernel<MODE, NT, OUT, NPAD>;
   static DeviceOnce once;
   const int dev = current_device();
   if (once.need(dev)) {
@@ -585,23 +681,24 @@
     if ((rc = make_map(&maps.m[0], a.in_hi, a.in_lo, a.CIN, a.ID, a.IH, a.IW, 1, 1, 0, 0, G::PC, G::PR))) return rc;
     maps.m[1] = maps.m[2] = maps.m[3] = maps.m[0];
   }
-  const int tiles_w = cdiv(OW, 8 * NT), tiles_h = cdiv(OH, 16);
+  const int tiles_w = cdiv(cells_w, 8 * NT), tiles_h = cdiv(cells_h, 16);
   const long long nitems = (long long)tiles_w * tiles_h * cdiv(a.ID, DC);
   MVSF_REQUIRE(nitems < (1ll << 30), "conv3d_tc: volume too large");
   const int grid = (int)(nitems < num_sms ? nitems : num_sms);
-  kern<<<grid, c3::THREADS, smem, s>>>(maps, a, NS, wres, OH, OW, tiles_w, tiles_h, DC, (int)nitems);
+  kern<<<grid, c3::THREADS, smem, s>>>(maps, a, NS, wres, cells_h, cells_w, tiles_w, tiles_h, DC, (int)nitems);
   MVSF_LAUNCH_CHECK("conv3d_col");
   return MVSF_OK;
 }
 
-template <int MODE>
+template <int MODE, int OUT>
 static int launch_col(const ConvTcArgs& a, cudaStream_t s) {
+  constexpr bool DEC = MODE == DECONV_S2;
   const int D = a.ID;
-  const int OH = MODE == CONV_S1 ? a.IH : (a.IH - 1) / 2 + 1, OW = MODE == CONV_S1 ? a.IW : (a.IW - 1) / 2 + 1;
+  const int OH = MODE == CONV_S2 ? (a.IH - 1) / 2 + 1 : a.IH, OW = MODE == CONV_S2 ? (a.IW - 1) / 2 + 1 : a.IW;
   const int num_sms = device_sm_count(current_device());
   const int NPAD = c3::npad(a.COUT);
   const int ngroups = a.CIN / 8 / a.KG;
-  const size_t slab = (size_t)NPAD * 1728;
+  const size_t slab = (size_t)NPAD * (DEC ? 3072 : 1728);
   const size_t wres_bytes = align_up(ngroups * slab, 128);
   const int wres = wres_bytes <= 112 * 1024 ? 1 : 0;
   int best_nt = 0, best_dc = 0, best_ns = 0;
@@ -610,7 +707,7 @@
   const int nts[3] = {4, 2, 1};
   for (int k = 0; k < 3; ++k) {
     const int nt = nts[k];
-    if (3 * nt * NPAD > 128) continue;
+    if (DEC ? nt != 1 : 3 * nt * NPAD > 128) continue;
     const uint32_t oct = nt == 4 ? c3::Geo<MODE, 4>::OCT_BYTES : (nt == 2 ? c3::Geo<MODE, 2>::OCT_BYTES : c3::Geo<MODE, 1>::OCT_BYTES);
     const size_t stage = align_up((size_t)a.KG * oct + (wres ? 0 : slab), 128);
     const size_t fixed = (wres ? wres_bytes : 0) + 256;
@@ -629,11 +726,17 @@
     }
   }
   MVSF_REQUIRE(best_nt > 0, "conv3d_col: no tile shape fits (CIN %d COUT %d)", a.CIN, a.COUT);
-  if (NPAD == 16) {
-    if (best_nt == 2) return launch_col_one<MODE, 2, 16>(a, best_ns, wres, best_smem, OH, OW, best_dc, num_sms, s);
-    return launch_col_one<MODE, 1, 16>(a, best_ns, wres, best_smem, OH, OW, best_dc, num_sms, s);
-  }
-  return launch_col_one<MODE, 1, 32>(a, best_ns, wres, best_smem, OH, OW, best_dc, num_sms, s);
+  if constexpr (DEC) {
+    MVSF_REQUIRE(NPAD == 16, "conv3d_col: transposed convs stream with COUT <= 16 only");
+    return launch_col_one<MODE, 1, OUT, 16>(a, best_ns, wres, best_smem, OH, OW, best_dc, num_sms, s);
+  } else {
+    static_assert(OUT == OUT_SPLIT, "the depth-streaming convs write fp16 hi|lo activations");
+    if (NPAD == 16) {
+      if (best_nt == 2) return launch_col_one<MODE, 2, OUT, 16>(a, best_ns, wres, best_smem, OH, OW, best_dc, num_sms, s);
+      return launch_col_one<MODE, 1, OUT, 16>(a, best_ns, wres, best_smem, OH, OW, best_dc, num_sms, s);
+    }
+    return launch_col_one<MODE, 1, OUT, 32>(a, best_ns, wres, best_smem, OH, OW, best_dc, num_sms, s);
+  }
 }
 
 int launch_conv3d_tc(const ConvTcArgs& a, int mode, int out_mode, cudaStream_t s) {
@@ -644,17 +747,22 @@
   MVSF_REQUIRE(a.KG == conv3d_tc_kg(mode, a.CIN), "conv3d_tc: KG must be conv3d_tc_kg(mode, CIN) (it fixes the weight slab layout)");
   MVSF_REQUIRE(((uintptr_t)a.in_hi & 15) == 0 && ((uintptr_t)a.in_lo & 15) == 0 && ((uintptr_t)a.wtc & 15) == 0,
                "conv3d_tc: operands must be 16-byte aligned");
-  MVSF_REQUIRE(a.col == conv3d_tc_col(mode, a.SD, a.COUT), "conv3d_tc: col must be conv3d_tc_col(mode, SD, COUT) (weight slab layout)");
+  MVSF_REQUIRE(a.col == 0 || a.col == conv3d_tc_col(mode, a.SD, a.COUT),
+               "conv3d_tc: col must be conv3d_tc_col(mode, SD, COUT), or 0 for the per-slice kernel (weight slab layout)");
   if (out_mode == OUT_SPLIT) {
     MVSF_REQUIRE(a.out_hi && a.out_lo, "conv3d_tc: split output missing");
-    if (a.col) return mode == CONV_S1 ? launch_col<CONV_S1>(a, s) : launch_col<CONV_S2>(a, s);
+    if (a.col) {
+      if (mode == CONV_S1) return launch_col<CONV_S1, OUT_SPLIT>(a, s);
+      if (mode == CONV_S2) return launch_col<CONV_S2, OUT_SPLIT>(a, s);
+      return launch_col<DECONV_S2, OUT_SPLIT>(a, s);
+    }
     if (mode == CONV_S1) return launch_mode<CONV_S1, OUT_SPLIT>(a, s);
     if (mode == CONV_S2) return launch_mode<CONV_S2, OUT_SPLIT>(a, s);
     if (mode == DECONV_S2) return launch_mode<DECONV_S2, OUT_SPLIT>(a, s);
   } else if (mode == DECONV_S2 && (out_mode == OUT_F32 || out_mode == OUT_PROB)) {
     MVSF_REQUIRE(a.out32 && a.skip32 && a.COUT == 8 && (out_mode == OUT_F32 || a.probw), "conv3d_tc: fp32 output needs out32, skip32, COUT == 8");
-    if (out_mode == OUT_F32) return launch_mode<DECONV_S2, OUT_F32>(a, s);
-    return launch_mode<DECONV_S2, OUT_PROB>(a, s);
+    if (out_mode == OUT_F32) return a.col ? launch_col<DECONV_S2, OUT_F32>(a, s) : launch_mode<DECONV_S2, OUT_F32>(a, s);
+    return a.col ? launch_col<DECONV_S2, OUT_PROB>(a, s) : launch_mode<DECONV_S2, OUT_PROB>(a, s);
   }
   return fail(MVSF_ERR_INVALID, "conv3d_tc: unsupported mode %d / output %d", mode, out_mode);
 }
@@ -663,11 +771,14 @@
 
 using namespace mvsf;
 
-extern "C" int mvsf_conv3d_tc_layer(int mode, int sd, const float* in, const float* w32, const float* skip, float* out,
-                                    void* workspace, size_t workspace_bytes, int cin, int cout, int ID, int IH, int IW,
-                                    mvsf_stream_t stream) {
+static int conv3d_tc_layer(int mode, int sd, int out_mode, int col, const float* in, const float* w32, const float* skip,
+                           const float* probw, float* out, void* workspace, size_t workspace_bytes, int cin, int cout,
+                           int ID, int IH, int IW, cudaStream_t s) {
   MVSF_REQUIRE(in && w32 && out && workspace && (mode >= 0 && mode <= 2) && (sd == 1 || sd == 2), "conv3d_tc_layer: bad arguments");
   MVSF_REQUIRE(cin % 8 == 0 && cout % 8 == 0, "conv3d_tc_layer: channels must be multiples of 8");
+  MVSF_REQUIRE(out_mode == OUT_SPLIT || (mode == DECONV_S2 && skip && (out_mode == OUT_F32 || (out_mode == OUT_PROB && probw))),
+               "conv3d_tc_layer: fp32 outputs are those of a transposed conv with an fp32 skip (and prob weights)");
+  MVSF_REQUIRE(col == 0 || col == conv3d_tc_col(mode, sd, cout), "conv3d_tc_layer: this layer has no depth-streaming kernel");
   int OD, OH, OW;
   if (mode == CONV_S1) { OD = ID; OH = IH; OW = IW; }
   else if (mode == CONV_S2) { OD = (ID - 1) / sd + 1; OH = (IH - 1) / 2 + 1; OW = (IW - 1) / 2 + 1; }
@@ -676,21 +787,39 @@
   const size_t nw = align_up(conv3d_tc_packed_halves(mode, cin, cout), 64);
   const size_t need = (2 * nin + 4 * nout + nw) * sizeof(__half) + 256;
   if (workspace_bytes < need) return fail(MVSF_ERR_WORKSPACE, "conv3d_tc_layer: workspace %zu < %zu bytes", workspace_bytes, need);
-  cudaStream_t s = (cudaStream_t)stream;
   __half* xin = reinterpret_cast<__half*>(workspace);
   __half* xout = xin + 2 * nin;
   __half* xskip = xout + 2 * nout;
   __half* wtc = xskip + 2 * nout;
   int rc;
   if ((rc = launch_split_f16(in, nin, xin, 2 * nin, 1, nin, s))) return rc;
-  if (skip && (rc = launch_split_f16(skip, nout, xskip, 2 * nout, 1, nout, s))) return rc;
-  if ((rc = conv3d_tc_pack(w32, wtc, mode, sd, cin, cout, s))) return rc;
+  if (out_mode == OUT_SPLIT && skip && (rc = launch_split_f16(skip, nout, xskip, 2 * nout, 1, nout, s))) return rc;
+  if ((rc = conv3d_tc_pack(w32, wtc, mode, col, cin, cout, s))) return rc;
   ConvTcArgs a{};
   a.in_hi = xin; a.in_lo = xin + nin; a.wtc = wtc; a.bias = w32 + (size_t)27 * cin * cout;
+  a.CIN = cin; a.COUT = cout; a.SD = sd; a.ID = ID; a.IH = IH; a.IW = IW; a.KG = conv3d_tc_kg(mode, cin);
+  a.col = col;
+  if (out_mode != OUT_SPLIT) {
+    a.skip32 = skip; a.out32 = out; a.probw = probw;
+    return launch_conv3d_tc(a, mode, out_mode, s);
+  }
   if (skip) { a.skip_hi = xskip; a.skip_lo = xskip + nout; }
   a.out_hi = xout; a.out_lo = xout + nout;
-  a.CIN = cin; a.COUT = cout; a.SD = sd; a.ID = ID; a.IH = IH; a.IW = IW; a.KG = conv3d_tc_kg(mode, cin);
-  a.col = conv3d_tc_col(mode, sd, cout);
   if ((rc = launch_conv3d_tc(a, mode, OUT_SPLIT, s))) return rc;
   return launch_merge_vec8(xout, xout + nout, out, nout, s);
 }
+
+extern "C" int mvsf_conv3d_tc_layer(int mode, int sd, const float* in, const float* w32, const float* skip, float* out,
+                                    void* workspace, size_t workspace_bytes, int cin, int cout, int ID, int IH, int IW,
+                                    mvsf_stream_t stream) {
+  return conv3d_tc_layer(mode, sd, OUT_SPLIT, conv3d_tc_col(mode, sd, cout), in, w32, skip, nullptr, out, workspace,
+                         workspace_bytes, cin, cout, ID, IH, IW, (cudaStream_t)stream);
+}
+
+extern "C" int mvsf_conv3d_tc_layer_out(int mode, int sd, int out_mode, int col, const float* in, const float* w32,
+                                        const float* skip, const float* probw, float* out, void* workspace,
+                                        size_t workspace_bytes, int cin, int cout, int ID, int IH, int IW,
+                                        mvsf_stream_t stream) {
+  return conv3d_tc_layer(mode, sd, out_mode, col, in, w32, skip, probw, out, workspace, workspace_bytes, cin, cout, ID, IH,
+                         IW, (cudaStream_t)stream);
+}
diff --git a/mvsformerplusplus_b200/csrc/conv3d_tc.cuh b/mvsformerplusplus_b200/csrc/conv3d_tc.cuh
--- a/mvsformerplusplus_b200/csrc/conv3d_tc.cuh
+++ b/mvsformerplusplus_b200/csrc/conv3d_tc.cuh
@@ -25,7 +25,7 @@
 int conv3d_tc_kg(int mode, int cin);
 size_t conv3d_tc_packed_halves(int mode, int cin, int cout);
 int conv3d_tc_col(int mode, int sd, int cout);
-int conv3d_tc_pack(const float* w32, __half* out, int mode, int sd, int cin, int cout, cudaStream_t s);
+int conv3d_tc_pack(const float* w32, __half* out, int mode, int col, int cin, int cout, cudaStream_t s);
 int launch_conv3d_tc(const ConvTcArgs& a, int mode, int out_mode, cudaStream_t s);
 int launch_merge_vec8(const __half* hi, const __half* lo, float* x, size_t n, cudaStream_t s);
 
diff --git a/mvsformerplusplus_b200/csrc/costreg_unet.cu b/mvsformerplusplus_b200/csrc/costreg_unet.cu
--- a/mvsformerplusplus_b200/csrc/costreg_unet.cu
+++ b/mvsformerplusplus_b200/csrc/costreg_unet.cu
@@ -103,6 +103,7 @@
     a.wtc = w16[8]; a.bias = bias[8];
     a.skip32 = vol;
     a.CIN = 16; a.COUT = 8; a.SD = SD; a.ID = D1; a.IH = H1; a.IW = W1; a.KG = conv3d_tc_kg(DECONV_S2, 16);
+    a.col = conv3d_tc_col(DECONV_S2, SD, 8);
     if (kind == 1) {
       a.out32 = logits; a.probw = wp;
       if ((rc = launch_conv3d_tc(a, DECONV_S2, OUT_PROB, s))) return rc;
@@ -148,7 +149,8 @@
   const float* p = conv;
   __half* q = reinterpret_cast<__half*>(wts_tc);
   for (int l = 0; l < 9; ++l) {
-    int rc = conv3d_tc_pack(p, q, kLayerMode[l], kind == 0 ? 2 : 1, kLayerCh[l][0], kLayerCh[l][1], (cudaStream_t)stream);
+    const int col = conv3d_tc_col(kLayerMode[l], kind == 0 ? 2 : 1, kLayerCh[l][1]);
+    int rc = conv3d_tc_pack(p, q, kLayerMode[l], col, kLayerCh[l][0], kLayerCh[l][1], (cudaStream_t)stream);
     if (rc) return rc;
     p += (size_t)27 * kLayerCh[l][0] * kLayerCh[l][1];
     q += conv3d_tc_packed_halves(kLayerMode[l], kLayerCh[l][0], kLayerCh[l][1]);
```

Measured after the change: 51.91 (median of 6 runs). 1.6% higher.
